# starreeze/drin

Measured on AMD Instinct MI355X. Metric: mention x candidate pairs scored/sec, higher is better.
Workload: dtype bf16x3; 1 GPU; wikimel-shaped scoring forward: 100-cand (+1 answer slot), D=768, R=2048, L=128, P=49, T=64 token-level entity text; parallelism=dp1 (mentions sharded, no collective)

## Files before the change

drin_amd/_lib.py:

```python
from __future__ import annotations

import ctypes as C
import os
from typing import Optional

_HERE = os.path.dirname(os.path.abspath(__file__))
LIB_PATH = os.environ.get("DRIN_LIB_PATH") or os.path.join(_HERE, "libdrin_hip.so")
MAX_LAYERS = 8
ABI_VERSION = 12

OK, E_SHAPE, E_NULL, E_ALIGN, E_WORKSPACE, E_HIP, E_UNSUPPORTED, E_INDEX = 0, -1, -2, -3, -4, -5, -6, -7
PREC_F32, PREC_BF16X3, PREC_BF16X3_ALL, PREC_BF16X3_IF16 = 0, 1, 3, 5
FEAT_F32, FEAT_BF16 = 0, 1
CACHE_F32, CACHE_MIXED_F16 = 0, 1
CACHE_FORMATS = {"f32": CACHE_F32, "mixed_f16": CACHE_MIXED_F16}
ACTIVATIONS = {"gelu": 1, "sigmoid": 2, "relu": 3, "tanh": 4, "silu": 5}

fp = C.POINTER(C.c_float)
ip = C.POINTER(C.c_int64)


class DrinConfigC(C.Structure):
    _fields_ = [
        ("batch", C.c_int32), ("num_candidates", C.c_int32), ("embed_dim", C.c_int32), ("image_dim", C.c_int32),
        ("mention_tokens", C.c_int32), ("image_regions", C.c_int32), ("mention_objects", C.c_int32),
        ("entity_objects", C.c_int32), ("entity_tokens", C.c_int32), ("mention_object_inner", C.c_int32),
        ("entity_image_inner", C.c_int32), ("entity_object_inner", C.c_int32), ("num_layers", C.c_int32),
        ("dynamic_edges", C.c_int32), ("edge_enabled", C.c_float * 4), ("layer_norm_eps", C.c_float),
        ("cosine_eps", C.c_float), ("miei_eps", C.c_float), ("clip_scale", C.c_float), ("precision", C.c_int32),
        ("num_entities", C.c_int32), ("vector_edges", C.c_int32), ("feature_dtype", C.c_int32),
        ("vertex_activation", C.c_int32), ("edge_activation", C.c_int32), ("cache_format", C.c_int32),
    ]


class DrinBatchC(C.Structure):
    _fields_ = [
        ("mention_text", C.c_void_p), ("mention_start", C.c_void_p), ("mention_end", C.c_void_p),
        ("mention_image", C.c_void_p), ("mention_object", C.c_void_p), ("mention_object_score", C.c_void_p),
        ("entity_text", C.c_void_p), ("entity_text_mask", C.c_void_p), ("entity_image", C.c_void_p),
        ("entity_object", C.c_void_p), ("entity_object_score", C.c_void_p), ("miet_similarity", C.c_void_p),
        ("mtei_similarity", C.c_void_p), ("entity_index", C.c_void_p), ("entity_text_cls", C.c_void_p),
        ("index_status", C.c_void_p),
    ]


class DrinLayerParamsC(C.Structure):
    _fields_ = [(n, C.c_void_p) for n in ("w_h", "b_h", "w_u", "b_u", "w_v", "b_v", "ln_weight", "ln_bias", "w_m", "b_m")]


class DrinParamsC(C.Structure):
    _fields_ = [(n, C.c_void_p) for n in (
        "w_mention_text", "b_mention_text", "w_entity_text", "b_entity_text",
        "w_mention_image", "b_mention_image", "w_entity_image", "b_entity_image")] + [("layer", DrinLayerParamsC * MAX_LAYERS)]


class DrinParamGradsC(C.Structure):
    _fields_ = DrinParamsC._fields_


class DrinInputGradsC(C.Structure):
    _fields_ = [(n, C.c_void_p) for n in (
        "mention_text", "mention_image", "mention_object", "mention_object_score", "entity_text", "entity_text_cls",
        "entity_image", "entity_object", "entity_object_score", "miet_similarity", "mtei_similarity", "scratch")] + [
        ("scratch_bytes", C.c_size_t)]


class DrinMelhiConfigC(C.Structure):
    _fields_ = [("batch", C.c_int32), ("num_candidates", C.c_int32), ("embed_dim", C.c_int32), ("image_dim", C.c_int32),
                ("mention_tokens", C.c_int32), ("image_regions", C.c_int32), ("precision", C.c_int32),
                ("cosine_eps", C.c_float), ("thres_tmim", C.c_float), ("thres_imie", C.c_float)]


class DrinMelhiBatchC(C.Structure):
    _fields_ = [(n, C.c_void_p) for n in (
        "mention_feature", "mention_mask", "start", "end", "mention_image", "entity_feature", "entity_image")]


MELHI_PARAMS = ("w_image_map_text", "b_image_map_text", "w_ih", "w_hh", "b_ih", "b_hh", "w_mention_final_map",
                "b_mention_final_map", "w_entity_final_map", "b_entity_final_map")


class DrinMelhiParamsC(C.Structure):
    _fields_ = [(n, C.c_void_p) for n in MELHI_PARAMS]


class DrinMelhiParamGradsC(C.Structure):
    _fields_ = DrinMelhiParamsC._fields_


class DrinGhmfcConfigC(C.Structure):
    _fields_ = [("batch", C.c_int32), ("num_candidates", C.c_int32), ("embed_dim", C.c_int32), ("image_dim", C.c_int32),
                ("mention_tokens", C.c_int32), ("image_regions", C.c_int32), ("num_heads", C.c_int32),
                ("entity_tokens", C.c_int32), ("precision", C.c_int32), ("layer_norm_eps", C.c_float), ("cosine_eps", C.c_float)]


class DrinGhmfcBatchC(C.Structure):
    _fields_ = [(n, C.c_void_p) for n in ("mention_feature", "mention_mask", "mention_image", "entity_feature", "entity_mask")]


GHMFC_CROSS_PARAMS = ("a2b_wq", "a2b_wk", "a2b_wv", "a2b_in_bias", "a2b_wo", "a2b_bo", "a2b_ffn_w", "a2b_ffn_b", "b2a_in_w",
                      "b2a_in_bias", "b2a_wo", "b2a_bo", "b2a_ffn_w", "b2a_ffn_b", "ln0_w", "ln0_b", "ln1_w", "ln1_b", "ln2_w",
                      "ln2_b", "ln3_w", "ln3_b")


class DrinGhmfcCrossParamsC(C.Structure):
    _fields_ = [(n, C.c_void_p) for n in GHMFC_CROSS_PARAMS]


class DrinGhmfcParamsC(C.Structure):
    _fields_ = [("t2v", DrinGhmfcCrossParamsC), ("v2t", DrinGhmfcCrossParamsC)] + [(n, C.c_void_p) for n in (
        "w_text_linear", "b_text_linear", "w_image_linear", "b_image_linear", "w_score_linear", "b_score_linear", "w_entity",
        "b_entity")]


class DrinTraceC(C.Structure):
    _fields_ = [(n, C.c_void_p * (MAX_LAYERS + 1)) for n in (
        "mention_text_vertex", "mention_image_vertex", "entity_text_vertex", "entity_image_vertex", "edges")]


EXPORTS = {
    "drin_version": (C.c_int, []),
    "drin_last_error": (C.c_char_p, []),
    "drin_build_info": (C.c_char_p, []),
    "drin_default_config": (C.c_int, [C.POINTER(DrinConfigC)]),
    "drin_host_selftest": (C.c_int, []),
    "drin_workspace_bytes": (C.c_size_t, [C.POINTER(DrinConfigC), C.c_int]),
    "drin_edges_fwd": (C.c_int, [C.POINTER(DrinConfigC), C.POINTER(DrinBatchC), C.c_void_p, C.c_void_p, C.c_void_p]),
    "drin_pool_fwd": (C.c_int, [C.POINTER(DrinConfigC), C.POINTER(DrinBatchC), C.c_void_p, C.c_void_p, C.c_void_p, C.c_void_p]),
    "drin_linear_fwd": (C.c_int, [C.c_void_p, C.c_void_p, C.c_void_p, C.c_void_p, C.c_int64, C.c_int32, C.c_int32, C.c_int32, C.c_void_p]),
    "drin_linear_bwd": (C.c_int, [C.c_void_p, C.c_void_p, C.c_void_p, C.c_void_p, C.c_void_p, C.c_void_p, C.c_int64, C.c_int32,
                                  C.c_int32, C.c_int32, C.c_void_p, C.c_size_t, C.c_void_p]),
    "drin_forward": (C.c_int, [C.POINTER(DrinConfigC), C.POINTER(DrinBatchC), C.POINTER(DrinParamsC), C.c_void_p,
                               C.c_size_t, C.c_void_p, C.c_int, C.POINTER(DrinTraceC), C.c_void_p]),
    "drin_forward_staged": (C.c_int, [C.POINTER(DrinConfigC), C.POINTER(DrinBatchC), C.POINTER(DrinParamsC), C.c_void_p,
                                      C.c_size_t, C.c_void_p, C.c_int, C.POINTER(DrinTraceC), C.c_void_p, C.c_void_p]),
    "drin_backward": (C.c_int, [C.POINTER(DrinConfigC), C.POINTER(DrinBatchC), C.POINTER(DrinParamsC), C.c_void_p,
                                C.c_size_t, C.c_void_p, C.POINTER(DrinParamGradsC), C.c_void_p]),
    "drin_backward_staged": (C.c_int, [C.POINTER(DrinConfigC), C.POINTER(DrinBatchC), C.POINTER(DrinParamsC), C.c_void_p,
                                       C.c_size_t, C.c_void_p, C.POINTER(DrinParamGradsC), C.c_void_p, C.c_void_p]),
    "drin_backward_ex": (C.c_int, [C.POINTER(DrinConfigC), C.POINTER(DrinBatchC), C.POINTER(DrinParamsC), C.c_void_p,
                                   C.c_size_t, C.c_void_p, C.POINTER(DrinParamGradsC), C.POINTER(DrinInputGradsC), C.c_void_p,
                                   C.c_void_p]),
    "drin_input_grad_scratch_bytes": (C.c_size_t, [C.POINTER(DrinConfigC)]),
    "drin_pool_bwd": (C.c_int, [C.POINTER(DrinConfigC), C.c_void_p, C.c_void_p, C.c_void_p, C.c_void_p, C.c_void_p]),
    "drin_fused_supported": (C.c_int, [C.POINTER(DrinConfigC)]),
    "drin_indexed_supported": (C.c_int, [C.POINTER(DrinConfigC)]),
    "drin_prepared_bytes": (C.c_size_t, [C.POINTER(DrinConfigC)]),
    "drin_fused_workspace_bytes": (C.c_size_t, [C.POINTER(DrinConfigC)]),
    "drin_workgroups_per_mention": (C.c_int32, [C.POINTER(DrinConfigC), C.c_int32]),
    "drin_index_status": (C.c_int, [C.c_void_p, C.c_void_p]),
    "drin_image_contraction_passes": (C.c_int32, [C.POINTER(DrinConfigC), C.c_int32]),
    "drin_prepare": (C.c_int, [C.POINTER(DrinConfigC), C.POINTER(DrinParamsC), C.c_void_p, C.c_size_t, C.c_void_p]),
    "drin_forward_prepared": (C.c_int, [C.POINTER(DrinConfigC), C.POINTER(DrinBatchC), C.POINTER(DrinParamsC), C.c_void_p,
                                        C.c_void_p, C.c_size_t, C.c_void_p, C.c_void_p]),
    "drin_entity_cache_bytes": (C.c_size_t, [C.POINTER(DrinConfigC)]),
    "drin_entity_cache_build_workspace_bytes": (C.c_size_t, [C.POINTER(DrinConfigC)]),
    "drin_cached_workspace_bytes": (C.c_size_t, [C.POINTER(DrinConfigC)]),
    "drin_build_entity_cache": (C.c_int, [C.POINTER(DrinConfigC), C.POINTER(DrinBatchC), C.POINTER(DrinParamsC), C.c_void_p,
                                          C.c_void_p, C.c_size_t, C.c_void_p, C.c_size_t, C.c_void_p]),
    "drin_forward_cached": (C.c_int, [C.POINTER(DrinConfigC), C.POINTER(DrinBatchC), C.POINTER(DrinParamsC), C.c_void_p,
                                      C.c_void_p, C.c_void_p, C.c_size_t, C.c_void_p, C.c_void_p]),
    "drin_split_planes": (C.c_int, [C.c_void_p, C.c_void_p, C.c_void_p, C.c_int64, C.c_void_p]),
    "drin_linear_planes_fwd": (C.c_int, [C.c_void_p, C.c_void_p, C.c_void_p, C.c_void_p, C.c_void_p, C.c_void_p,
                                         C.c_int64, C.c_int32, C.c_int32, C.c_void_p]),
    "drin_loss_workspace_bytes": (C.c_size_t, [C.c_int32]),
    "drin_triplet_topk": (C.c_int, [C.c_void_p, C.c_void_p, C.c_int32, C.c_int32, C.c_float, C.POINTER(C.c_int32), C.c_int32,
                                    C.c_void_p, C.c_void_p, C.c_void_p, C.c_void_p, C.c_size_t, C.c_void_p]),
    "drin_adam_step": (C.c_int, [C.c_void_p, C.c_void_p, C.c_void_p, C.c_void_p, C.c_int64, C.c_float, C.c_float, C.c_float,
                                 C.c_float, C.c_float, C.c_float, C.c_void_p]),
    "drin_melhi_workspace_bytes": (C.c_size_t, [C.POINTER(DrinMelhiConfigC), C.c_int]),
    "drin_melhi_forward": (C.c_int, [C.POINTER(DrinMelhiConfigC), C.POINTER(DrinMelhiBatchC), C.POINTER(DrinMelhiParamsC), C.c_void_p,
                                     C.c_void_p, C.c_void_p, C.c_size_t, C.c_void_p, C.c_void_p]),
    "drin_melhi_backward": (C.c_int, [C.POINTER(DrinMelhiConfigC), C.POINTER(DrinMelhiBatchC), C.POINTER(DrinMelhiParamsC),
                                      C.c_void_p, C.c_void_p, C.c_void_p, C.c_size_t, C.c_void_p, C.POINTER(DrinMelhiParamGradsC),
                                      C.c_void_p]),
    "drin_ghmfc_workspace_bytes": (C.c_size_t, [C.POINTER(DrinGhmfcConfigC)]),
    "drin_ghmfc_forward": (C.c_int, [C.POINTER(DrinGhmfcConfigC), C.POINTER(DrinGhmfcBatchC), C.POINTER(DrinGhmfcParamsC), C.c_void_p,
                                     C.c_size_t, C.c_void_p, C.c_void_p, C.c_void_p]),
    "drin_attention": (C.c_int, [C.c_void_p, C.c_int64, C.c_void_p, C.c_int64, C.c_void_p, C.c_int64, C.c_void_p, C.c_void_p, C.c_int64,
                                 C.c_int32, C.c_int32, C.c_int32, C.c_int32, C.c_int32, C.c_void_p]),
    "drin_attention_train_fwd": (C.c_int, [C.c_void_p, C.c_int64, C.c_void_p, C.c_int64, C.c_void_p, C.c_int64, C.c_void_p, C.c_void_p,
                                           C.c_int64, C.c_void_p, C.c_int32, C.c_int32, C.c_int32, C.c_int32, C.c_int32, C.c_void_p]),
    "drin_attention_bwd": (C.c_int, [C.c_void_p, C.c_int64, C.c_void_p, C.c_int64, C.c_void_p, C.c_int64, C.c_void_p, C.c_void_p,
                                     C.c_int64, C.c_void_p, C.c_void_p, C.c_int64, C.c_void_p, C.c_int64, C.c_void_p, C.c_int64,
                                     C.c_void_p, C.c_int64, C.c_void_p, C.c_int32, C.c_int32, C.c_int32, C.c_int32, C.c_int32,
                                     C.c_void_p]),
    "drin_profile_begin": (C.c_int, [C.c_int]),
    "drin_profile_end": (C.c_int, [C.POINTER(C.c_double), C.POINTER(C.c_int64)]),
    "drin_kernel_class_name": (C.c_char_p, [C.c_int]),
}
KERNEL_CLASSES = 12


class DrinError(RuntimeError):
    def __init__(self, status: int, message: str):
        super().__init__(f"libdrin_hip status {status}: {message}")
        self.status = status


_lib: Optional[C.CDLL] = None


def load() -> C.CDLL:
    global _lib
    if _lib is not None:
        return _lib
    if not os.path.exists(LIB_PATH):
        raise ImportError(
            f"{LIB_PATH} is missing: the DRIN HIP path has no fallback. Build it with `python -m drin_amd.build`."
        )
    try:
        import torch
    except ImportError:
        pass
    lib = C.CDLL(LIB_PATH)
    for name, (res, args) in EXPORTS.items():
        fn = getattr(lib, name)
        fn.restype, fn.argtypes = res, args
    if lib.drin_version() != ABI_VERSION:
        raise ImportError(f"libdrin_hip ABI {lib.drin_version()} != binding {ABI_VERSION}; rebuild")
    _lib = lib
    return lib


def profile_begin(max_launches: int = 65536) -> None:
    check(load().drin_profile_begin(max_launches))


def profile_end() -> dict:
    ms = (C.c_double * KERNEL_CLASSES)()
    n = (C.c_int64 * KERNEL_CLASSES)()
    check(load().drin_profile_end(ms, n))
    lib = load()
    return {lib.drin_kernel_class_name(k).decode(): (ms[k], n[k]) for k in range(KERNEL_CLASSES)}


def check(status: int) -> None:
    if status != OK:
        raise DrinError(status, load().drin_last_error().decode())
```

drin_amd/csrc/api.hip:

```cpp
#include <dlfcn.h>
#include <stdarg.h>
#include <stdlib.h>

#include <atomic>
#include <mutex>
#include <stdio.h>
#include <string.h>

#include "fused.h"
#include "internal.h"
#include "layout.h"

namespace drin {

static thread_local char g_err[512] = "";

void set_error(const char* fmt, ...) {
  va_list ap;
  va_start(ap, fmt);
  vsnprintf(g_err, sizeof(g_err), fmt, ap);
  va_end(ap);
}

int hip_fail(hipError_t e, const char* what) {
  set_error("%s: %s", what, hipGetErrorString(e));
  return DRIN_E_HIP;
}

static thread_local int g_call_device = -1;

int call_device() {
  if (g_call_device >= 0) return g_call_device;
  int dev = 0;
  if (hipGetDevice(&dev) != hipSuccess) dev = 0;
  return dev;
}

DeviceScope::DeviceScope(void* stream, const void* device_pointer, const char* entry_point)
    : status(DRIN_OK), prev(-1), dev(-1), outer(g_call_device), switched(false) {
  hipError_t e = hipGetDevice(&prev);
  if (e != hipSuccess) {
    (void)hipGetLastError();
    prev = -1;
    return;
  }
  dev = prev;
  if (stream != nullptr) {
    hipDevice_t d = 0;
    e = hipStreamGetDevice((hipStream_t)stream, &d);
    if (e != hipSuccess) {
      set_error("%s: hipStreamGetDevice: %s (is `stream` a hipStream_t?)", entry_point, hipGetErrorString(e));
      status = DRIN_E_HIP;
      return;
    }
    dev = (int)d;
  } else if (device_pointer != nullptr) {
    hipPointerAttribute_t attr;
    if (hipPointerGetAttributes(&attr, device_pointer) == hipSuccess && attr.type == hipMemoryTypeDevice)
      dev = attr.device;
    else
      (void)hipGetLastError();
  }
  if (dev != prev) {
    e = hipSetDevice(dev);
    if (e != hipSuccess) {
      set_error("%s: hipSetDevice(%d): %s", entry_point, dev, hipGetErrorString(e));
      status = DRIN_E_HIP;
      return;
    }
    switched = true;
  }
  g_call_device = dev;
}

DeviceScope::~DeviceScope() {
  if (status != DRIN_OK || prev < 0) return;
  g_call_device = outer;
  if (switched) (void)hipSetDevice(prev);
}

struct Roctx {
  int (*push)(const char*) = nullptr;
  int (*pop)() = nullptr;
  Roctx() {
    if (!getenv("DRIN_ROCTX")) return;
    void* h = dlopen("librocprofiler-sdk-roctx.so", RTLD_NOW | RTLD_GLOBAL);
    if (!h) h = dlopen("libroctx64.so", RTLD_NOW | RTLD_GLOBAL);
    if (!h) return;
    push = reinterpret_cast<int (*)(const char*)>(dlsym(h, "roctxRangePushA"));
    pop = reinterpret_cast<int (*)()>(dlsym(h, "roctxRangePop"));
    if (!push || !pop) push = nullptr, pop = nullptr;
  }
};
static const Roctx& roctx() {
  static const Roctx r;
  return r;
}
RoctxRange::RoctxRange(const char* name) : pushed(false) {
  const Roctx& r = roctx();
  if (r.push) {
    r.push(name);
    pushed = true;
  }
}
RoctxRange::~RoctxRange() {
  if (pushed) roctx().pop();
}

struct Profile {
  std::atomic<bool> open{false};
  int capacity = 0;
  std::atomic<int> used{0};
  hipEvent_t* start = nullptr;
  hipEvent_t* stop = nullptr;
  int* cls = nullptr;
};
static Profile g_prof;
static std::mutex g_prof_mutex;

KernelTimer::KernelTimer(int kernel_class, hipStream_t st) : slot(-1), stream(st) {
  Profile& p = g_prof;
  if (!p.open.load(std::memory_order_acquire)) return;
  const int s = p.used.fetch_add(1, std::memory_order_relaxed);
  if (s >= p.capacity) return;
  slot = s;
  p.cls[slot] = kernel_class;
  (void)hipEventRecord(p.start[slot], st);
}

KernelTimer::~KernelTimer() {
  if (slot >= 0) (void)hipEventRecord(g_prof.stop[slot], stream);
}

static void profile_free(Profile& p) {
  for (int i = 0; i < p.capacity; ++i) {
    if (p.start) (void)hipEventDestroy(p.start[i]);
    if (p.stop) (void)hipEventDestroy(p.stop[i]);
  }
  delete[] p.start;
  delete[] p.stop;
  delete[] p.cls;
  p.start = p.stop = nullptr;
  p.cls = nullptr;
  p.capacity = 0;
  p.used.store(0);
  p.open.store(false);
}

int vertex_act(const drin_config* c) { return c->vertex_activation == DRIN_ACT_DEFAULT ? DRIN_ACT_GELU : c->vertex_activation; }
int edge_act(const drin_config* c) { return c->edge_activation == DRIN_ACT_DEFAULT ? DRIN_ACT_SIGMOID : c->edge_activation; }

int validate_config(const drin_config* c) {
  if (!c) {
    set_error("config is NULL");
    return DRIN_E_NULL;
  }
  if (c->batch < 0 || c->num_candidates <= 0 || c->embed_dim <= 0 || c->image_dim <= 0 || c->mention_tokens <= 0 ||
      c->image_regions <= 0 || c->mention_objects < 0 || c->entity_objects < 0 || c->entity_tokens < 0 ||
      c->mention_object_inner < 0 || c->entity_image_inner < 0 || c->entity_object_inner < 0) {
    set_error("config: negative or zero dimension");
    return DRIN_E_SHAPE;
  }
  if (c->embed_dim % 4 || c->image_dim % 4) {
    set_error("config: embed_dim=%d and image_dim=%d must be multiples of 4 (16-byte lane accesses)", c->embed_dim,
              c->image_dim);
    return DRIN_E_SHAPE;
  }
  if (c->embed_dim > 1024) {
    set_error("config: embed_dim=%d > 1024 is not built (LayerNorm row kept in registers)", c->embed_dim);
    return DRIN_E_UNSUPPORTED;
  }
  if (c->vector_edges && (c->embed_dim % 8)) {
    set_error("config: vector edges need embed_dim %% 8 == 0 (got %d)", c->embed_dim);
    return DRIN_E_SHAPE;
  }
  if (c->num_layers < 0 || c->num_layers > DRIN_MAX_LAYERS) {
    set_error("config: num_layers=%d outside [0, %d]", c->num_layers, DRIN_MAX_LAYERS);
    return DRIN_E_SHAPE;
  }
  if ((int64_t)c->batch * c->num_candidates > (int64_t)1 << 30) {
    set_error("config: batch * num_candidates too large for one call; split the batch");
    return DRIN_E_SHAPE;
  }
  if (c->feature_dtype != DRIN_FEAT_F32 && c->feature_dtype != DRIN_FEAT_BF16) {
    set_error("config: feature_dtype %d is not DRIN_FEAT_F32 / DRIN_FEAT_BF16", c->feature_dtype);
    return DRIN_E_UNSUPPORTED;
  }
  if (c->vertex_activation < DRIN_ACT_DEFAULT || c->vertex_activation > DRIN_ACT_SILU) {
    set_error("config: vertex_activation %d is not a drin_activation", c->vertex_activation);
    return DRIN_E_UNSUPPORTED;
  }
  if (c->edge_activation < DRIN_ACT_DEFAULT || c->edge_activation > DRIN_ACT_SILU) {
    set_error("config: edge_activation %d is not a drin_activation", c->edge_activation);
    return DRIN_E_UNSUPPORTED;
  }
  if (c->cache_format != DRIN_CACHE_F32 && c->cache_format != DRIN_CACHE_MIXED_F16) {
    set_error("config: cache_format %d is not a drin_cache_format", c->cache_format);
    return DRIN_E_UNSUPPORTED;
  }
  if (c->precision != DRIN_PREC_F32 && c->precision != DRIN_PREC_BF16X3 && c->precision != DRIN_PREC_BF16X3_ALL &&
      c->precision != DRIN_PREC_BF16X3_IF16) {
    set_error("config: precision %d is not a drin_precision", c->precision);
    return DRIN_E_UNSUPPORTED;
  }
  return DRIN_OK;
}

static int validate_batch(const drin_config* c, const drin_batch* b) {
  if (!b) {
    set_error("batch is NULL");
    return DRIN_E_NULL;
  }
  if (c->feature_dtype != DRIN_FEAT_F32) {
    set_error("bf16 feature storage is read by drin_forward_prepared only; widen the features to fp32 for this entry point");
    return DRIN_E_UNSUPPORTED;
  }
  if (c->precision == DRIN_PREC_BF16X3_IF16) {
    set_error("DRIN_PREC_BF16X3_IF16 (the entity-image contraction in one fp16 pass) is an inference mode of drin_forward_prepared; use DRIN_PREC_BF16X3 here");
    return DRIN_E_UNSUPPORTED;
  }
  const void* req[] = {b->mention_text,  b->mention_start,        b->mention_end,     b->mention_image,
                       b->mention_object, b->mention_object_score, b->entity_text,     b->entity_image,
                       b->entity_object,  b->entity_object_score,  b->miet_similarity, b->mtei_similarity};
  const char* names[] = {"mention_text",   "mention_start",        "mention_end",     "mention_image",
                         "mention_object", "mention_object_score", "entity_text",     "entity_image",
                         "entity_object",  "entity_object_score",  "miet_similarity", "mtei_similarity"};
  for (int i = 0; i < 12; ++i) {
    if (!req[i]) {
      set_error("batch.%s is NULL", names[i]);
      return DRIN_E_NULL;
    }
  }
  if (c->entity_tokens > 0 && !b->entity_text_mask) {
    set_error("batch.entity_text_mask is NULL but entity_tokens=%d", c->entity_tokens);
    return DRIN_E_NULL;
  }
  if (b->entity_text_cls && c->entity_tokens > 0) {
    set_error("batch.entity_text_cls goes with pooled entity text (entity_tokens = 0), not with a token block");
    return DRIN_E_UNSUPPORTED;
  }
  const void* al[] = {b->mention_text, b->mention_image, b->mention_object, b->entity_text, b->entity_image,
                      b->entity_object, b->entity_text_cls};
  for (const void* p : al)
    if (!aligned16(p)) {
      set_error("batch: feature tensors must be 16-byte aligned");
      return DRIN_E_ALIGN;
    }
  return DRIN_OK;
}

static int validate_params(const drin_config* c, const drin_params* p) {
  if (!p) {
    set_error("params is NULL");
    return DRIN_E_NULL;
  }
  const void* req[] = {p->w_mention_text,  p->b_mention_text,  p->w_entity_text,  p->b_entity_text,
                       p->w_mention_image, p->b_mention_image, p->w_entity_image, p->b_entity_image};
  for (const void* q : req)
    if (!q || !aligned16(q)) {
      set_error("params: vertex encoder tensor NULL or not 16-byte aligned");
      return q ? DRIN_E_ALIGN : DRIN_E_NULL;
    }
  for (int l = 0; l < c->num_layers; ++l) {
    const drin_layer_params& L = p->layer[l];
    const void* lr[] = {L.w_h, L.b_h, L.w_u, L.b_u, L.w_v, L.b_v, L.ln_weight, L.ln_bias};
    for (const void* q : lr)
      if (!q || !aligned16(q)) {
        set_error("params: layer %d tensor NULL or not 16-byte aligned", l);
        return q ? DRIN_E_ALIGN : DRIN_E_NULL;
      }
    if (c->vector_edges && (!L.w_m || !L.b_m || !aligned16(L.w_m) || !aligned16(L.b_m))) {
      set_error("params: layer %d w_m / b_m (vector edges, model.py:112) NULL or not 16-byte aligned", l);
      return DRIN_E_NULL;
    }
  }
  return DRIN_OK;
}

static Pooled unpooled(const drin_config* c, const drin_batch* b, const float* span_mean) {
  Pooled p;
  p.span_mean = span_mean;
  p.mention_object = b->mention_object;
  p.entity_object = b->entity_object;
  p.entity_image = b->entity_image;
  p.entity_text = b->entity_text;
  p.entity_text_raw_stride = c->entity_tokens > 0 ? (int64_t)c->entity_tokens * c->embed_dim : c->embed_dim;
  return p;
}

void resolve_pooled(const drin_config* c, const drin_batch* b, const Layout& L, float* ws, Pooled* out) {
  *out = unpooled(c, b, ws + L.span_mean);
  out->mention_image = ws + L.mimg_pool;
  if (c->mention_object_inner > 1) out->mention_object = ws + L.mobj_pool;
  if (c->entity_object_inner > 1) out->entity_object = ws + L.eobj_pool;
  if (c->entity_image_inner > 1) out->entity_image = ws + L.eimg_pool;
  if (c->entity_tokens > 0) out->entity_text = ws + L.xet_pool;
}

int run_pooling(const drin_config* c, const drin_batch* b, const Layout& L, float* ws, Pooled* out, hipStream_t st) {
  const int B = c->batch, N = c->num_candidates, D = c->embed_dim, R = c->image_dim;
  const int64_t M = (int64_t)B * N;
  resolve_pooled(c, b, L, ws, out);
  auto copy_of = [](const float* resolved, const float* raw) { return resolved != raw ? const_cast<float*>(resolved) : nullptr; };
  DRIN_TRY(launch_span_mean(b->mention_text, b->mention_start, b->mention_end, ws + L.span_mean, B, c->mention_tokens, D, st));
  DRIN_TRY(launch_axis_mean(b->mention_image, ws + L.mimg_pool, B, c->image_regions, R, st));
  if (float* dst = copy_of(out->mention_object, b->mention_object))
    DRIN_TRY(launch_axis_mean(b->mention_object, dst, (int64_t)B * c->mention_objects, c->mention_object_inner, R, st));
  if (float* dst = copy_of(out->entity_object, b->entity_object))
    DRIN_TRY(launch_axis_mean(b->entity_object, dst, M * c->entity_objects, c->entity_object_inner, R, st));
  if (float* dst = copy_of(out->entity_image, b->entity_image))
    DRIN_TRY(launch_axis_mean(b->entity_image, dst, M, c->entity_image_inner, R, st));
  if (float* dst = copy_of(out->entity_text, b->entity_text))
    DRIN_TRY(launch_entity_token_mean(b->entity_text, b->entity_text_mask, dst, M, c->entity_tokens, D, st));
  return DRIN_OK;
}

int run_static_edges(const drin_config* c, const drin_batch* b, const Pooled& P, float* edges, hipStream_t st) {
  const int B = c->batch, N = c->num_candidates;
  const int64_t M = (int64_t)B * N;
  const float* raw = b->entity_text_cls ? b->entity_text_cls : b->entity_text;
  const int64_t raw_stride = b->entity_text_cls ? (int64_t)c->embed_dim : P.entity_text_raw_stride;
  DRIN_TRY(launch_cosine_rows(P.span_mean, raw, raw_stride, edges + 0 * M, B, N, c->embed_dim, c->cosine_eps, 1.0f, st,
                              b->entity_index, b->mtei_similarity, b->miet_similarity, edges + 1 * M, edges + 2 * M,
                              c->clip_scale));
  DRIN_TRY(launch_miei(P.mention_object, b->mention_object_score, P.entity_object, b->entity_object_score,
                       edges + 3 * M, B, N, c->mention_objects, c->entity_objects, c->image_dim, c->cosine_eps,
                       c->miei_eps, 1.0f, st, b->entity_index));
  return DRIN_OK;
}

static int copy_out(float* dst, const float* src, size_t n, hipStream_t st) {
  if (!dst) return DRIN_OK;
  hipError_t e = hipMemcpyAsync(dst, src, n * sizeof(float), hipMemcpyDeviceToDevice, st);
  if (e != hipSuccess) return hip_fail(e, "hipMemcpyAsync(trace)");
  return DRIN_OK;
}

static int tap(const drin_trace* t, int l, const Layout& L, const float* ws, int B, int64_t M, int D, hipStream_t st,
               size_t edge_width = 1) {
  if (!t) return DRIN_OK;
  DRIN_TRY(copy_out(t->mention_text_vertex[l], ws + L.vm[l], (size_t)B * D, st));
  DRIN_TRY(copy_out(t->mention_image_vertex[l], ws + L.vm[l] + (size_t)B * D, (size_t)B * D, st));
  DRIN_TRY(copy_out(t->entity_text_vertex[l], ws + L.ve[l], (size_t)M * D, st));
  DRIN_TRY(copy_out(t->entity_image_vertex[l], ws + L.ve[l] + (size_t)M * D, (size_t)M * D, st));
  DRIN_TRY(copy_out(t->edges[l], ws + L.edges[l], (size_t)4 * M * edge_width, st));
  return DRIN_OK;
}

static int indexed_supported(const drin_config* c, const char* who) {
  const int64_t M = (int64_t)c->batch * c->num_candidates;
  const int D = c->embed_dim, R = c->image_dim;
  const bool x3 = c->precision == DRIN_PREC_BF16X3 || c->precision == DRIN_PREC_BF16X3_ALL;
  if (c->num_entities <= 0 || c->entity_tokens != 0 || c->entity_image_inner > 1 || c->entity_object_inner > 1 ||
      c->entity_objects != 1 || c->vector_edges || !x3 || M < 1024 || (D % 32) || (R % 32) || D < 128 || R < 128 ||
      R > 2048 || c->batch > 65535) {
    set_error("%s: entity_index needs pooled entity text tables (entity_tokens = 0, num_entities > 0), one object per entity, "
              "inner dims <= 1, scalar edges, split-bf16 precision, D and R multiples of 32 (>= 128, R <= 2048) and at least "
              "1024 pairs; gather on the caller side otherwise", who);
    return DRIN_E_UNSUPPORTED;
  }
  return DRIN_OK;
}

struct InputGradScratch {
  size_t total_floats = 0;
  size_t g_span = 0, g_raw = 0, cls_stage = 0, g_pool = 0, cos3 = 0, g_mimg = 0, g_eimg = 0, g_mobj = 0, g_eobj = 0;
  size_t g_ms = 0, g_es = 0, g_edge = 0, planes_ei = 0, planes_et = 0, miei = 0;
  size_t take(size_t n) {
    const size_t o = total_floats;
    total_floats += (n + 63) & ~(size_t)63;
    return o;
  }
  void build(const drin_config& c) {
    const size_t B = (size_t)c.batch, N = (size_t)c.num_candidates, D = (size_t)c.embed_dim, R = (size_t)c.image_dim;
    const size_t M = B * N, Km = (size_t)c.mention_objects, Ke = (size_t)c.entity_objects;
    const bool x3 = c.precision == DRIN_PREC_BF16X3 || c.precision == DRIN_PREC_BF16X3_ALL;
    total_floats = 0;
    g_span = take(B * D);
    g_raw = take(M * D);
    cls_stage = take(c.entity_tokens > 0 ? M * D : 0);
    g_pool = take(c.entity_tokens > 0 ? M * D : 0);
// ... 870 lines not shown
```

drin_amd/csrc/fused_forward.hip:

```cpp
#include <string.h>

#include "fused.h"
#include "internal.h"
#include "layout.h"

namespace drin {

constexpr int kMixedMinCandidates = 64;

struct FusedLayout {
  size_t span_mean, mimg, vm0, hmfu, q, e0m, e1m, xt, s_part, s_text, s_img, sig, tm, tm2, agg1, vm1, hm2, h_text, h_image,
      et1, s2_part, agg2, mt2, p_xt, p_xi, p_et1, xi_scale, splitk, splitk_floats, pair_splitk, pair_splitk_floats, total;
  int chunks;
  void build(const drin_config& c) {
    const size_t B = c.batch, N = c.num_candidates, D = c.embed_dim, R = c.image_dim, M = B * N;
    chunks = (int)(B >= 2048 ? (N + 127) / 128 : B >= 1024 ? (N + 47) / 48 : (N + 15) / 16);
    size_t off = 0;
    auto take = [&off](size_t n) {
      const size_t o = off;
      off += (n + 63) & ~(size_t)63;
      return o;
    };
    span_mean = take(B * D);
    mimg = take(B * R);
    vm0 = take(2 * B * D);
    hmfu = take(2 * B * 2 * D);
    q = take(2 * B * (D + R));
    e0m = take(4 * M);
    e1m = take(4 * M);
    xt = take(c.entity_tokens > 0 ? M * D : 0);
    s_part = take(B * chunks * (2 * D + 2 * R + 4));
    s_text = take(2 * B * D);
    s_img = take(2 * B * R);
    sig = take(4 * B);
    tm = take(2 * B * D);
    tm2 = take(2 * B * D);
    agg1 = take(2 * B * D);
    vm1 = take(2 * B * D);
    hm2 = take(2 * B * D);
    h_text = take(M * D);
    h_image = take(M * D);
    et1 = take(M * D);
    s2_part = take(B * chunks * 2 * D);
    agg2 = take(B * D);
    mt2 = take(B * D);
    const bool planes = c.precision == DRIN_PREC_BF16X3 || c.precision == DRIN_PREC_BF16X3_ALL || c.precision == DRIN_PREC_BF16X3_IF16;
    p_xt = take(planes ? M * D : 0);
    p_xi = take(!planes ? 0 : c.num_entities > 0 ? M * R : c.precision == DRIN_PREC_BF16X3_IF16 ? M * R / 2 : 0);
    p_et1 = take(planes ? M * D : 0);
    xi_scale = take(c.precision == DRIN_PREC_BF16X3_IF16 ? M : 0);
    splitk_floats = 2 * B <= 512 ? 8 * 2 * B * (D + R) : 0;
    if (planes && splitk_floats < (size_t)192 * 65536) splitk_floats = (size_t)192 * 65536;
    splitk = take(splitk_floats);
    pair_splitk_floats = 0;
    {
      const size_t tiles = ((M + 255) / 256) * ((D + 255) / 256);
      if (planes && tiles <= 128)
        for (size_t s : {16, 8, 6, 4, 3, 2})
          if (tiles * s <= 256) {
            pair_splitk_floats = s * ((M + 255) / 256 * 256) * D;
            break;
          }
    }
    pair_splitk = take(pair_splitk_floats);
    total = off;
  }
};

static bool if16_gate(const drin_config* c, bool indexed) {
  const int64_t M = (int64_t)c->batch * c->num_candidates;
  return c->precision == DRIN_PREC_BF16X3_IF16 && !indexed && c->feature_dtype == DRIN_FEAT_F32 &&
         c->num_candidates >= kMixedMinCandidates && c->embed_dim == 768 && c->image_dim == 2048 &&
         cdiv(M, 256) * cdiv(c->embed_dim, 256) >= 128;
}

int fused_supported(const drin_config* c) {
  if (c->num_layers != 2) {
    set_error("fused path: built for num_layers == 2 (got %d); use drin_forward", c->num_layers);
    return DRIN_E_UNSUPPORTED;
  }
  if (c->vector_edges) {
    set_error("fused path: vector edge features (model.py:112-116) run on the layer-by-layer path; use drin_forward");
    return DRIN_E_UNSUPPORTED;
  }
  if (c->mention_object_inner > 1 || c->entity_object_inner > 1 || c->entity_image_inner > 1) {
    set_error("fused path: inner feature dims > 1 need the pooled path of drin_forward");
    return DRIN_E_UNSUPPORTED;
  }
  const bool tiny = c->embed_dim <= 256 && c->image_dim <= 256;
  const bool full = c->embed_dim <= 768 && c->image_dim <= 2048;
  if (!tiny && !full) {
    set_error("fused path: D=%d R=%d outside the built instantiations", c->embed_dim, c->image_dim);
    return DRIN_E_UNSUPPORTED;
  }
  return DRIN_OK;
}

}

using namespace drin;

extern "C" {

int drin_split_planes(const float* x, void* hi, void* lo, int64_t n, void* stream) {
  DRIN_BIND_DEVICE(stream, x, "drin_split_planes");
  if (!x || !hi || !lo) {
    set_error("drin_split_planes: NULL argument");
    return DRIN_E_NULL;
  }
  return launch_split_planes(x, hi, lo, n, (hipStream_t)stream);
}

int drin_linear_planes_fwd(const void* x_hi, const void* x_lo, const void* w_hi, const void* w_lo, const float* bias,
                           float* y, int64_t rows, int32_t n_out, int32_t k, void* stream) {
  DRIN_BIND_DEVICE(stream, y, "drin_linear_planes_fwd");
  if (!x_hi || !w_hi || !w_lo || !y) {
    set_error("drin_linear_planes_fwd: NULL argument");
    return DRIN_E_NULL;
  }
  return launch_gemm_x3_planes(x_hi, x_lo, k, w_hi, w_lo, k, bias, y, n_out, rows, n_out, k, (hipStream_t)stream);
}

int drin_fused_supported(const drin_config* cfg) {
  DRIN_TRY(validate_config(cfg));
  return fused_supported(cfg);
}

size_t drin_prepared_bytes(const drin_config* cfg) {
  if (validate_config(cfg) != DRIN_OK || fused_supported(cfg) != DRIN_OK) return 0;
  Prepared P;
  P.build(*cfg);
  return P.total * sizeof(float);
}

int drin_prepare(const drin_config* cfg, const drin_params* params, void* prepared, size_t prepared_bytes,
                 void* stream) {
  DRIN_BIND_DEVICE(stream, prepared, "drin_prepare");
  RoctxRange range("drin_prepare");
  DRIN_TRY(validate_config(cfg));
  DRIN_TRY(fused_supported(cfg));
  if (!params || !prepared) {
    set_error("drin_prepare: NULL argument");
    return DRIN_E_NULL;
  }
  Prepared P;
  P.build(*cfg);
  if (prepared_bytes < P.total * sizeof(float) || !aligned16(prepared)) {
    set_error("drin_prepare: buffer has %zu bytes (needs %zu) or is not 16-byte aligned", prepared_bytes,
              P.total * sizeof(float));
    return DRIN_E_WORKSPACE;
  }
  hipStream_t st = (hipStream_t)stream;
  float* pb = (float*)prepared;
  const int D = cfg->embed_dim, R = cfg->image_dim;
  const drin_layer_params& L1 = params->layer[0];
  const int F32 = DRIN_PREC_F32;
  auto copy = [&](float* dst, const float* src, size_t n) -> int {
    hipError_t e = hipMemcpyAsync(dst, src, n * sizeof(float), hipMemcpyDeviceToDevice, st);
    return e == hipSuccess ? DRIN_OK : hip_fail(e, "hipMemcpyAsync(prepare)");
  };
  DRIN_TRY(copy(pb + P.wcat1, L1.w_h, (size_t)D * D));
  DRIN_TRY(copy(pb + P.wcat1 + (size_t)D * D, L1.w_u, (size_t)D * D));
  {
    hipError_t e = hipMemsetAsync(pb + P.bcat1, 0, D * sizeof(float), st);
    if (e != hipSuccess) return hip_fail(e, "hipMemsetAsync(prepare)");
  }
  DRIN_TRY(copy(pb + P.bcat1 + D, L1.b_u, D));
  DRIN_TRY(launch_gemm_nn(L1.w_v, D, params->w_entity_text, D, pb + P.etmp, D + R, D, D, D, false, F32, st));
  DRIN_TRY(launch_gemm_nn(L1.w_v, D, params->w_entity_image, R, pb + P.etmp + D, D + R, D, R, D, false, F32, st));
  DRIN_TRY(launch_transpose(pb + P.etmp, pb + P.ecat, D, D + R, st));
  DRIN_TRY(launch_gemm_nt(params->b_entity_text, D, L1.w_v, D, L1.b_v, pb + P.k_t, D, 1, D, D, false, F32, st));
  DRIN_TRY(launch_gemm_nt(params->b_entity_image, D, L1.w_v, D, L1.b_v, pb + P.k_i, D, 1, D, D, false, F32, st));
  DRIN_TRY(launch_gemm_nn(L1.w_h, D, params->w_entity_text, D, pb + P.c_txt, D, D, D, D, false, F32, st));
  DRIN_TRY(launch_gemm_nn(L1.w_h, D, params->w_entity_image, R, pb + P.c_img, R, D, R, D, false, F32, st));
  DRIN_TRY(launch_gemm_nt(params->b_entity_text, D, L1.w_h, D, L1.b_h, pb + P.cb_t, D, 1, D, D, false, F32, st));
  DRIN_TRY(launch_gemm_nt(params->b_entity_image, D, L1.w_h, D, L1.b_h, pb + P.cb_i, D, 1, D, D, false, F32, st));
  {
    const size_t dd = (size_t)D * D, dr = (size_t)D * R;
    __bf16* q = reinterpret_cast<__bf16*>(pb + P.p_ctxt);
    DRIN_TRY(launch_split_planes(pb + P.c_txt, q, q + dd, dd, st));
    q = reinterpret_cast<__bf16*>(pb + P.p_cimg);
    DRIN_TRY(launch_split_planes(pb + P.c_img, q, q + dr, dr, st));
    DRIN_TRY(launch_to_f16_scaled(pb + P.c_img, pb + P.p_cimg_f16, (int64_t)dr, pb + P.cimg_f16_scale, st));
    q = reinterpret_cast<__bf16*>(pb + P.p_wh2);
    DRIN_TRY(launch_split_planes(params->layer[1].w_h, q, q + dd, dd, st));
    struct { size_t off; const float* w; size_t n; } extra[] = {
        {P.p_wmt, params->w_mention_text, dd},  {P.p_wmi, params->w_mention_image, dr},
        {P.p_wcat1, pb + P.wcat1, 2 * dd},      {P.p_ecat, pb + P.ecat, dd + dr},
        {P.p_wet, params->w_entity_text, dd},   {P.p_wei, params->w_entity_image, dr},
        {P.p_wh1, L1.w_h, dd}};
    for (const auto& e : extra) {
      q = reinterpret_cast<__bf16*>(pb + e.off);
      DRIN_TRY(launch_split_planes(e.w, q, q + e.n, e.n, st));
    }
  }
  return DRIN_OK;
}

}

namespace drin {

static int folded_precision(const drin_config* c) { return c->precision == DRIN_PREC_BF16X3_IF16 ? (int)DRIN_PREC_BF16X3 : c->precision; }

int run_folded_head(const drin_config* cfg, const drin_batch* b, const drin_params* params, const float* pb, const Prepared& P,
                    bool weight_planes, float* span_mean, float* mimg, float* vm0, float* hmfu, GemmScratch sk, hipStream_t st) {
  const int B = cfg->batch, D = cfg->embed_dim, R = cfg->image_dim, prec = folded_precision(cfg);
  auto wp = [&](size_t plane_off) -> const float* { return weight_planes ? pb + plane_off : nullptr; };
  if (cfg->feature_dtype == DRIN_FEAT_BF16) {
    DRIN_TRY(launch_span_mean_bf16(b->mention_text, b->mention_start, b->mention_end, span_mean, B, cfg->mention_tokens, D, st));
    DRIN_TRY(launch_axis_mean_bf16(b->mention_image, mimg, B, cfg->image_regions, R, st));
  } else {
    DRIN_TRY(launch_span_mean(b->mention_text, b->mention_start, b->mention_end, span_mean, B, cfg->mention_tokens, D, st));
    DRIN_TRY(launch_axis_mean(b->mention_image, mimg, B, cfg->image_regions, R, st));
  }
  DRIN_TRY(launch_gemm_nt_pair({span_mean, params->w_mention_text, params->b_mention_text, vm0, D, D, D, B, D, D, wp(P.p_wmt)},
                               {mimg, params->w_mention_image, params->b_mention_image, vm0 + (size_t)B * D, R, R, D, B, D, R, wp(P.p_wmi)},
                               prec, st, sk.p, sk.floats));
  return launch_gemm_nt(vm0, D, pb + P.wcat1, D, pb + P.bcat1, hmfu, 2 * D, 2 * (int64_t)B, 2 * D, D, false, prec, st, sk.p, sk.floats,
                        wp(P.p_wcat1));
}

int run_folded_mention_finish(const drin_config* cfg, const drin_params* params, const float* pb, const Prepared& P,
                              bool weight_planes, float* vm1, float* hm2, GemmScratch sk, hipStream_t st) {
  const int B = cfg->batch, D = cfg->embed_dim;
  const drin_layer_params& L1 = params->layer[0];
  DRIN_TRY(launch_layernorm_gelu(vm1, L1.ln_weight, L1.ln_bias, vm1, nullptr, nullptr, 2 * (int64_t)B, D, cfg->layer_norm_eps, st,
                                 vertex_act(cfg)));
  return launch_gemm_nt(vm1, D, params->layer[1].w_h, D, nullptr, hm2, D, 2 * (int64_t)B, D, D, false, folded_precision(cfg), st, sk.p,
                        sk.floats, weight_planes ? pb + P.p_wh2 : nullptr);
}

int run_folded_tail(const drin_config* cfg, const drin_params* params, const float* pb, const Prepared& P, int chunks,
                    const float* s2_part, const float* vm1, float* agg2, float* mt2, const float* hm2, const float* e1m, float* h2,
                    const float* et1, const void* et1_hi, bool weight_planes, GemmScratch sk, GemmScratch pair_sk, float* scores,
                    hipStream_t st) {
  const int B = cfg->batch, N = cfg->num_candidates, D = cfg->embed_dim, prec = folded_precision(cfg);
  const int64_t M = (int64_t)B * N;
  const drin_layer_params& L2 = params->layer[1];
  DRIN_TRY(launch_mention_input2(s2_part, vm1, agg2, B, D, N, chunks, st));
  DRIN_TRY(launch_gemm_nt(agg2, D, L2.w_h, D, L2.b_h, mt2, D, B, D, D, false, prec, st, sk.p, sk.floats,
                          weight_planes ? pb + P.p_wh2 : nullptr));
  DRIN_TRY(launch_layernorm_gelu(mt2, L2.ln_weight, L2.ln_bias, mt2, nullptr, nullptr, B, D, cfg->layer_norm_eps, st, vertex_act(cfg)));
  if (et1_hi) {
    const __bf16* e1 = static_cast<const __bf16*>(et1_hi);
    const __bf16* w2 = reinterpret_cast<const __bf16*>(pb + P.p_wh2);
    DRIN_TRY(launch_gemm_x3_planes(e1, e1 + (size_t)M * D, D, w2, w2 + (size_t)D * D, D, nullptr, h2, D, M, D, D, st, pair_sk.p,
                                   pair_sk.floats));
  } else {
    DRIN_TRY(launch_gemm_nt(et1, D, L2.w_h, D, nullptr, h2, D, M, D, D, false, prec, st));
  }
  FinalArgs fa = shaped_args<FinalArgs>(*cfg);
  set_vertex_fields(fa, *cfg);
  fa.h2 = h2;
  fa.hm2 = hm2;
  fa.b_h2 = L2.b_h;
  fa.gamma = L2.ln_weight;
  fa.beta = L2.ln_bias;
  fa.e1m = e1m;
  fa.mt2 = mt2;
  fa.scores = scores;
  fa.chunks = chunks;
  fa.cos_eps = cfg->cosine_eps;
  return launch_pair_final(fa, st);
}

static int forward_prepared_on_stream(const drin_config* cfg, const drin_batch* b, const drin_params* params, const void* prepared,
                                      void* workspace, float* scores, hipStream_t st) {
  FusedLayout L;
  L.build(*cfg);
  Prepared P;
  P.build(*cfg);
  float* ws = (float*)workspace;
  const float* pb = (const float*)prepared;
  const int B = cfg->batch, N = cfg->num_candidates, D = cfg->embed_dim, R = cfg->image_dim;
  const int64_t M = (int64_t)B * N;
  if (B == 0) return DRIN_OK;
  const int prec = folded_precision(cfg);
  const bool dyn = cfg->dynamic_edges != 0;
  const bool tokens = cfg->entity_tokens > 0;
  const bool planes = (prec == DRIN_PREC_BF16X3 || prec == DRIN_PREC_BF16X3_ALL) && (D % 32 == 0) && (R % 32 == 0);
  const bool indexed = b->entity_index != nullptr;
  const bool xi_planes = planes && indexed;
  const bool if16 = if16_gate(cfg, indexed) && gemm_f16_planes_fits(ws + L.p_xi, R, pb + P.p_cimg_f16, R, ws + L.h_image, D, M, D, R);
  if (b->entity_text_cls) {
    set_error("drin_forward_prepared: entity_text_cls (text pooled ahead of time) is a form of the training entry points");
    return DRIN_E_UNSUPPORTED;
  }
  if (indexed && cfg->num_entities <= 0) {
    set_error("drin_forward_prepared: entity_index given but cfg.num_entities = %d", cfg->num_entities);
    return DRIN_E_SHAPE;
  }
  if (indexed && !planes) {
    set_error("drin_forward_prepared: entity_index needs the split-bf16 precision (the stream kernel gathers the "
              "GEMM operands as planes); gather on the caller side for DRIN_PREC_F32");
    return DRIN_E_UNSUPPORTED;
  }
  const bool bf16_feat = cfg->feature_dtype == DRIN_FEAT_BF16;
  if (bf16_feat && !planes) {
    set_error("drin_forward_prepared: bf16 features need the split-bf16 precision (DRIN_PREC_BF16X3) and D, R multiples of 32");
    return DRIN_E_UNSUPPORTED;
  }
  __bf16* xt_hi = reinterpret_cast<__bf16*>(ws + L.p_xt);
  __bf16* xi_hi = reinterpret_cast<__bf16*>(ws + L.p_xi);
  __bf16* e1_hi = reinterpret_cast<__bf16*>(ws + L.p_et1);
  const size_t MD = (size_t)M * D, MR = (size_t)M * R;
  const drin_layer_params& L1 = params->layer[0];

  auto wp = [&](size_t plane_off) -> const float* { return planes ? pb + plane_off : nullptr; };
  const GemmScratch msk{L.splitk_floats ? ws + L.splitk : nullptr, L.splitk_floats};
  float* vm0 = ws + L.vm0;
  float* hmfu = ws + L.hmfu;
  const bool xt_exact = bf16_feat && !tokens;
  DRIN_TRY(run_folded_head(cfg, b, params, pb, P, planes, ws + L.span_mean, ws + L.mimg, vm0, hmfu, msk, st));
  if (dyn)
    DRIN_TRY(launch_gemm_nt(hmfu + D, 2 * D, pb + P.ecat, D, nullptr, ws + L.q, D + R, 2 * (int64_t)B, D + R, D, false, prec, st, msk.p,
                            msk.floats, wp(P.p_ecat)));
  StreamArgs sa = shaped_args<StreamArgs>(*cfg);
  set_edge_fields(sa, *cfg);
  sa.entity_text = b->entity_text;
  sa.entity_mask = b->entity_text_mask;
  sa.entity_image = b->entity_image;
  sa.entity_object = b->entity_object;
  sa.entity_object_score = b->entity_object_score;
  sa.entity_index = b->entity_index;
  sa.num_entities = cfg->num_entities;
  sa.index_status = b->index_status;
  sa.miet = b->miet_similarity;
  sa.mtei = b->mtei_similarity;
  sa.span_mean = ws + L.span_mean;
  sa.mobj = b->mention_object;
  sa.mscore = b->mention_object_score;
  sa.fu = hmfu + D;
  sa.ldfu = 2 * D;
  sa.q = ws + L.q;
  sa.ldq = D + R;
  sa.k_t = pb + P.k_t;
  sa.k_i = pb + P.k_i;
  sa.xt_out = planes ? nullptr : ws + L.xt;
  if (planes) {
    sa.xt_hi = xt_hi;
    sa.xt_lo = xt_exact ? nullptr : xt_hi + MD;
    if (xi_planes) {
      sa.xi_hi = xi_hi;
      sa.xi_lo = bf16_feat ? nullptr : xi_hi + MR;
    }
  }
  sa.xi_scale = if16 ? ws + L.xi_scale : nullptr;
  sa.xi_f16 = if16 ? static_cast<void*>(xi_hi) : nullptr;
  sa.e0m = ws + L.e0m;
  sa.e1m = ws + L.e1m;
  sa.s_part = ws + L.s_part;
  sa.T = cfg->entity_tokens;
  sa.Ke = cfg->entity_objects;
  sa.chunks = L.chunks;
  sa.bf16_features = bf16_feat ? 1 : 0;
  sa.s_text = ws + L.s_text;
  sa.s_img = ws + L.s_img;
  sa.sig = ws + L.sig;
  DRIN_TRY(launch_entity_stream(sa, st));
  if (L.chunks > 1)
    DRIN_TRY(launch_reduce_stream_partials(ws + L.s_part, ws + L.s_text, ws + L.s_img, ws + L.sig, B, D, R, L.chunks, st));
  DRIN_TRY(launch_gemm_nt_pair({ws + L.s_text, params->w_entity_text, nullptr, ws + L.tm, D, D, D, 2 * (int64_t)B, D, D, wp(P.p_wet)},
                               {ws + L.s_img, params->w_entity_image, nullptr, ws + L.tm2, R, R, D, 2 * (int64_t)B, D, R,
                                wp(P.p_wei)},
                               prec, st, msk.p, msk.floats));
  DRIN_TRY(launch_mention_input1(ws + L.tm, ws + L.tm2, ws + L.sig, params->b_entity_text, params->b_entity_image, vm0, ws + L.agg1, B, D, N, st));
  float* vm1 = ws + L.vm1;
  DRIN_TRY(launch_gemm_nt(ws + L.agg1, D, L1.w_h, D, L1.b_h, vm1, D, 2 * (int64_t)B, D, D, false, prec, st, msk.p, msk.floats, wp(P.p_wh1)));
  DRIN_TRY(run_folded_mention_finish(cfg, params, pb, P, planes, vm1, ws + L.hm2, msk, st));
  const GemmScratch psk = L.pair_splitk_floats ? GemmScratch{ws + L.pair_splitk, L.pair_splitk_floats} : msk;
  if (planes) {
    const __bf16* ct = reinterpret_cast<const __bf16*>(pb + P.p_ctxt);
    const __bf16* ci = reinterpret_cast<const __bf16*>(pb + P.p_cimg);
    DRIN_TRY(launch_gemm_x3_planes(xt_hi, xt_exact ? nullptr : xt_hi + MD, D, ct, ct + (size_t)D * D, D, nullptr, ws + L.h_text, D, M, D,
                                   D, st, psk.p, psk.floats));
    if (if16)
      DRIN_TRY(launch_gemm_f16_planes(xi_hi, R, pb + P.p_cimg_f16, R, ws + L.xi_scale, pb + P.cimg_f16_scale, ws + L.h_image, D, M, D, R,
                                      st, psk.p, psk.floats));
    else if (xi_planes)
      DRIN_TRY(launch_gemm_x3_planes(xi_hi, bf16_feat ? nullptr : xi_hi + MR, R, ci, ci + (size_t)D * R, R, nullptr, ws + L.h_image, D, M,
                                     D, R, st, psk.p, psk.floats));
    else if (bf16_feat)
      DRIN_TRY(launch_gemm_x3_planes(b->entity_image, nullptr, R, ci, ci + (size_t)D * R, R, nullptr, ws + L.h_image, D, M, D, R, st, psk.p,
                                     psk.floats));
    else
      DRIN_TRY(launch_gemm_nt_bf16x3(b->entity_image, R, pb + P.c_img, R, nullptr, ws + L.h_image, D, M, D, R, st, ci, ci + (size_t)D * R,
                                     false, psk.p, psk.floats));
  } else {
    const float* x_t = tokens ? ws + L.xt : b->entity_text;
    DRIN_TRY(launch_gemm_nt(x_t, D, pb + P.c_txt, D, nullptr, ws + L.h_text, D, M, D, D, false, prec, st));
    DRIN_TRY(launch_gemm_nt(b->entity_image, R, pb + P.c_img, R, nullptr, ws + L.h_image, D, M, D, R, false, prec, st));
  }
  PairArgs pa = shaped_args<PairArgs>(*cfg);
  set_vertex_fields(pa, *cfg);
  pa.h_text = ws + L.h_text;
  pa.h_image = ws + L.h_image;
  pa.hm = hmfu;
  pa.ldhm = 2 * D;
  pa.c_t = pb + P.cb_t;
  pa.c_i = pb + P.cb_i;
  pa.gamma = L1.ln_weight;
  pa.beta = L1.ln_bias;
  pa.e0m = ws + L.e0m;
  pa.e1m = ws + L.e1m;
  pa.et1 = planes ? nullptr : ws + L.et1;
  if (planes) {
    pa.et1_hi = e1_hi;
    pa.et1_lo = e1_hi + MD;
  }
  pa.s2_part = ws + L.s2_part;
  pa.chunks = L.chunks;
  DRIN_TRY(launch_pair_layer1(pa, st));
  return run_folded_tail(cfg, params, pb, P, L.chunks, ws + L.s2_part, vm1, ws + L.agg2, ws + L.mt2, ws + L.hm2, ws + L.e1m, ws + L.h_text,
                         planes ? nullptr : ws + L.et1, planes ? e1_hi : nullptr, planes, msk, psk, scores, st);
}

}

extern "C" {

int32_t drin_workgroups_per_mention(const drin_config* cfg, int32_t cached) {
  if (validate_config(cfg) != DRIN_OK || fused_supported(cfg) != DRIN_OK) return 0;
  if (cached) return cached_chunks_per_mention(*cfg);
  FusedLayout L;
  L.build(*cfg);
  return L.chunks;
}

int32_t drin_image_contraction_passes(const drin_config* cfg, int32_t indexed) {
  if (validate_config(cfg) != DRIN_OK || fused_supported(cfg) != DRIN_OK) return 0;
  if (cfg->precision == DRIN_PREC_F32) return 0;
  if (if16_gate(cfg, indexed != 0)) return 1;
  return cfg->feature_dtype == DRIN_FEAT_BF16 ? 2 : 3;
}

int drin_index_status(int32_t* index_status, void* stream) {
  if (!index_status) {
    set_error("drin_index_status: NULL argument");
    return DRIN_E_NULL;
  }
  DRIN_BIND_DEVICE(stream, index_status, "drin_index_status");
  int32_t w[4] = {0, 0, 0, 0};
  hipError_t e = hipMemcpyAsync(w, index_status, sizeof(w), hipMemcpyDeviceToHost, (hipStream_t)stream);
  if (e == hipSuccess) e = hipStreamSynchronize((hipStream_t)stream);
  if (e != hipSuccess) return hip_fail(e, "drin_index_status");
  if (w[0] == 0) return DRIN_OK;
  e = hipMemsetAsync(index_status, 0, sizeof(w), (hipStream_t)stream);
  if (e != hipSuccess) return hip_fail(e, "drin_index_status(reset)");
  const long long value = (long long)(((uint64_t)(uint32_t)w[3] << 32) | (uint32_t)w[2]);
  set_error("entity_index out of range: candidate row %lld at pair %d (b * N + n) is outside the entity tables - the row was clamped "
            "and a WRONG entity scored; drin/data.py:87-93 raises IndexError here", value, (int)w[1]);
  return DRIN_E_INDEX;
}

size_t drin_fused_workspace_bytes(const drin_config* cfg) {
  if (validate_config(cfg) != DRIN_OK || fused_supported(cfg) != DRIN_OK) return 0;
  FusedLayout L;
  L.build(*cfg);
  return L.total * sizeof(float);
}

int drin_forward_prepared(const drin_config* cfg, const drin_batch* b, const drin_params* params, const void* prepared,
                          void* workspace, size_t workspace_bytes, float* scores, void* stream) {
  DRIN_BIND_DEVICE(stream, workspace, "drin_forward_prepared");
  RoctxRange range("drin_forward_prepared");
  DRIN_TRY(validate_config(cfg));
  DRIN_TRY(fused_supported(cfg));
  if (!b || !params || !prepared || !workspace || !scores) {
    set_error("drin_forward_prepared: NULL argument");
    return DRIN_E_NULL;
  }
  FusedLayout L;
  L.build(*cfg);
  if (workspace_bytes < L.total * sizeof(float) || !aligned16(workspace)) {
    set_error("drin_forward_prepared: workspace has %zu bytes (needs %zu) or is not 16-byte aligned", workspace_bytes,
              L.total * sizeof(float));
    return DRIN_E_WORKSPACE;
  }
  return forward_prepared_on_stream(cfg, b, params, prepared, workspace, scores, (hipStream_t)stream);
}

}
```

drin_amd/csrc/gemm_x3_planes.hip:

```cpp
#include <stdlib.h>

#include "device_utils.h"
#include "internal.h"

namespace drin {

typedef float f32x16 __attribute__((ext_vector_type(16)));
typedef __bf16 bf16x8 __attribute__((ext_vector_type(8)));

namespace x3p {

constexpr int BM = 256, BN = 256, BK = 32;
constexpr int THREADS = 512;
constexpr int PLANE_BYTES = 256 * 64;
constexpr int BUF_BYTES = 4 * PLANE_BYTES;
constexpr int LDS_BYTES = 2 * BUF_BYTES;

__device__ __forceinline__ void tile_of_block(int& tile_x, int64_t& tile_y, int nx, unsigned full, int ksplit, int& kpart,
                                              unsigned& tail_slot) {
  const unsigned id = blockIdx.x;
  unsigned t;
  kpart = 0;
  tail_slot = 0;
  if (id < full) {
    const unsigned xcd = id & 7, k = id >> 3;
    const unsigned q = full >> 3, rem = full & 7;
    t = (xcd < rem ? xcd * (q + 1) : rem * (q + 1) + (xcd - rem) * q) + k;
  } else {
    const unsigned u = id - full;
    t = full + u / (unsigned)ksplit;
    kpart = (int)(u % (unsigned)ksplit);
    tail_slot = (u / (unsigned)ksplit) * (unsigned)(ksplit - 1) + (unsigned)(kpart - 1);
  }
  tile_x = (int)(t % (unsigned)nx);
  tile_y = (int64_t)(t / (unsigned)nx);
}

typedef __attribute__((address_space(1))) const void* gptr_t;
typedef __attribute__((address_space(3))) void* lptr_t;

struct Pieces {
  const char* base;
  int64_t ld_bytes;
  int64_t row0, lim;
};

template <bool A_LO, bool B_LO>
__device__ __forceinline__ void issue_piece(const Pieces& p, char* buf, int kb, int i) {
  const int wave = threadIdx.x >> 6;
  if (!A_LO && (wave >> 1) == 1) return;
  if (!B_LO && (wave >> 1) == 3) return;
  char* plane_base = buf + (wave >> 1) * PLANE_BYTES + (wave & 1) * 128 * 64;
  int64_t g = p.row0 + 16 * i;
  g = g < p.lim ? g : p.lim - 1;
  __builtin_amdgcn_global_load_lds((gptr_t)(p.base + g * p.ld_bytes + (int64_t)kb * (BK * 2)), (lptr_t)(plane_base + i * 1024),
                                   16, 0, 0);
}
template <bool A_LO, bool B_LO>
__device__ __forceinline__ void issue_tile(const Pieces& p, char* buf, int kb) {
#pragma unroll
  for (int i = 0; i < 8; ++i) issue_piece<A_LO, B_LO>(p, buf, kb, i);
}

typedef float f32x4 __attribute__((ext_vector_type(4)));

__device__ __forceinline__ int swz16(int row, int c) {
  const int f = (0x78 >> (((row >> 2) & 3) << 1)) & 3;
  return row * 64 + ((c ^ f) << 4);
}

__device__ __forceinline__ Pieces make_pieces(const __bf16* a_hi, const __bf16* a_lo, int64_t lda, int64_t m0,
                                                int64_t M, const __bf16* b_hi, const __bf16* b_lo, int64_t ldb,
                                                int64_t n0, int64_t N) {
  const int wave = threadIdx.x >> 6, lane = threadIdx.x & 63;
  const int plane = wave >> 1;
  const __bf16* base = plane == 0 ? a_hi : plane == 1 ? a_lo : plane == 2 ? b_hi : b_lo;
  const int64_t ld = plane < 2 ? lda : ldb, r0 = plane < 2 ? m0 : n0, lim = plane < 2 ? M : N;
  const int f = (0x78 >> (((lane >> 4) & 3) << 1)) & 3;
  const int chunk = (lane & 3) ^ f;
  Pieces p;
  p.base = reinterpret_cast<const char*>(base) + chunk * 16;
  p.ld_bytes = ld * 2;
  p.row0 = r0 + (wave & 1) * 128 + (lane >> 2);
  p.lim = lim;
  return p;
}

template <bool A_LO, bool B_LO>
__global__ void __launch_bounds__(THREADS, 2)
    k_gemm_x3_planes(const __bf16* __restrict__ a_hi, const __bf16* __restrict__ a_lo, int64_t lda,
                       const __bf16* __restrict__ b_hi, const __bf16* __restrict__ b_lo, int64_t ldb,
                       const float* __restrict__ bias, float* __restrict__ C, int64_t ldc, int64_t M, int N, int K,
                       int64_t part_stride, int nx, unsigned full, int ksplit, float* __restrict__ tail) {
  extern __shared__ __attribute__((aligned(16))) char smem[];
  if (gridDim.z > 1) {
    K /= (int)gridDim.z;
    const int64_t k0 = (int64_t)blockIdx.z * K;
    a_hi += k0;
    if (A_LO) a_lo += k0;
    b_hi += k0;
    if (B_LO) b_lo += k0;
    C += (int64_t)blockIdx.z * part_stride;
    ldc = N;
    bias = nullptr;
  }
  int tx, kpart;
  int64_t ty;
  unsigned tail_slot;
  tile_of_block(tx, ty, nx, full, ksplit, kpart, tail_slot);
  const int64_t m0 = ty * BM;
  const int n0 = tx * BN;
  if (blockIdx.x >= full) {
    K /= ksplit;
    const int64_t k0 = (int64_t)kpart * K;
    a_hi += k0;
    if (A_LO) a_lo += k0;
    b_hi += k0;
    if (B_LO) b_lo += k0;
  }
  const int nkb = K / BK;
  const int wave = threadIdx.x >> 6, lane = threadIdx.x & 63;
  const int wm = wave >> 2, wn = wave & 3;
  const int r = lane & 15, c = lane >> 4;

  f32x4 acc[8][4];
#pragma unroll
  for (int i = 0; i < 8; ++i)
#pragma unroll
    for (int j = 0; j < 4; ++j)
#pragma unroll
      for (int v = 0; v < 4; ++v) acc[i][j][v] = 0.f;

  const Pieces pieces = make_pieces(a_hi, A_LO ? a_lo : a_hi, lda, m0, M, b_hi, B_LO ? b_lo : b_hi, ldb, n0, N);
  issue_tile<A_LO, B_LO>(pieces, smem, 0);
  __syncthreads();

  for (int kb = 0; kb < nkb; ++kb) {
    const int cur = kb & 1;
    const char* buf = smem + cur * BUF_BYTES;
    const bool more = kb + 1 < nkb;
    char* nbuf = smem + (cur ^ 1) * BUF_BYTES;
    bf16x8 bh[4], bl[4], ah[2], al[2];
#pragma unroll
    for (int j = 0; j < 4; ++j) {
      const int off = swz16(wn * 64 + j * 16 + r, c);
      bh[j] = *reinterpret_cast<const bf16x8*>(buf + 2 * PLANE_BYTES + off);
      if (B_LO) bl[j] = *reinterpret_cast<const bf16x8*>(buf + 3 * PLANE_BYTES + off);
    }
    {
      const int off = swz16(wm * 128 + r, c);
      ah[0] = *reinterpret_cast<const bf16x8*>(buf + off);
      if (A_LO) al[0] = *reinterpret_cast<const bf16x8*>(buf + PLANE_BYTES + off);
    }
#pragma unroll
    for (int t = 0; t < 8; ++t) {
      if (more) issue_piece<A_LO, B_LO>(pieces, nbuf, kb + 1, t);
      if (t + 1 < 8) {
        const int off = swz16(wm * 128 + (t + 1) * 16 + r, c);
        ah[(t + 1) & 1] = *reinterpret_cast<const bf16x8*>(buf + off);
        if (A_LO) al[(t + 1) & 1] = *reinterpret_cast<const bf16x8*>(buf + PLANE_BYTES + off);
      }
      if (A_LO) {
#pragma unroll
        for (int j = 0; j < 4; ++j) acc[t][j] = __builtin_amdgcn_mfma_f32_16x16x32_bf16(bh[j], al[t & 1], acc[t][j], 0, 0, 0);
      }
      if (B_LO) {
#pragma unroll
        for (int j = 0; j < 4; ++j) acc[t][j] = __builtin_amdgcn_mfma_f32_16x16x32_bf16(bl[j], ah[t & 1], acc[t][j], 0, 0, 0);
      }
#pragma unroll
      for (int j = 0; j < 4; ++j) acc[t][j] = __builtin_amdgcn_mfma_f32_16x16x32_bf16(bh[j], ah[t & 1], acc[t][j], 0, 0, 0);
    }
    __syncthreads();
  }

  if (kpart > 0) {
    float* part = tail + (size_t)tail_slot * (BM * BN);
#pragma unroll
    for (int i = 0; i < 8; ++i)
#pragma unroll
      for (int j = 0; j < 4; ++j)
        st4(part + (wm * 128 + i * 16 + r) * BN + wn * 64 + j * 16 + c * 4,
            make_float4(acc[i][j][0], acc[i][j][1], acc[i][j][2], acc[i][j][3]));
    return;
  }
  const bool vec_ok = (ldc % 4) == 0 && (reinterpret_cast<uintptr_t>(C) & 15u) == 0;
#pragma unroll
  for (int i = 0; i < 8; ++i) {
    const int64_t row = m0 + wm * 128 + i * 16 + r;
    if (row >= M) continue;
#pragma unroll
    for (int j = 0; j < 4; ++j) {
      const int col = n0 + wn * 64 + j * 16 + c * 4;
      float* dst = C + row * ldc + col;
      if (vec_ok && col + 3 < N) {
        float4 o = make_float4(acc[i][j][0], acc[i][j][1], acc[i][j][2], acc[i][j][3]);
        if (bias != nullptr) o = o + ld4(bias + col);
        st4(dst, o);
      } else {
#pragma unroll
        for (int v = 0; v < 4; ++v)
          if (col + v < N) dst[v] = acc[i][j][v] + (bias != nullptr ? bias[col + v] : 0.f);
      }
    }
  }
}


__device__ __forceinline__ int pow2_exponent(float s) { return (int)((__builtin_bit_cast(uint32_t, s) >> 23) & 0xffu) - 127; }
__device__ __forceinline__ float4 scale_pow2(float4 v, int e) { return make_float4(ldexpf(v.x, e), ldexpf(v.y, e), ldexpf(v.z, e), ldexpf(v.w, e)); }

namespace p4 {

__device__ __forceinline__ void wait_units() { asm volatile("s_waitcnt vmcnt(4)" ::: "memory"); }
constexpr int UNIT_BYTES = 2 * 128 * 64;
constexpr int BUF = 4 * UNIT_BYTES;
constexpr int LDS = 2 * BUF;

struct Src {
  const char* ptr[4][2];
};

template <int U, int KB_BYTES = BK * 2>
__device__ __forceinline__ void issue_unit(const Src& s, char* buf, int kb) {
  const int wave = threadIdx.x >> 6;
  char* dst = buf + U * UNIT_BYTES + (wave >> 2) * (128 * 64) + (wave & 3) * 2048;
#pragma unroll
  for (int i = 0; i < 2; ++i)
    __builtin_amdgcn_global_load_lds((gptr_t)(s.ptr[U][i] + (int64_t)kb * KB_BYTES), (lptr_t)(dst + i * 1024), 16, 0, 0);
}

}

template <bool A_LO = true, bool F16 = false>
__global__ void __launch_bounds__(THREADS, 2)
    k_gemm_x3_planes_p4(const __bf16* __restrict__ a_hi, const __bf16* __restrict__ a_lo, int64_t lda,
                        const __bf16* __restrict__ b_hi, const __bf16* __restrict__ b_lo, int64_t ldb,
                        const float* __restrict__ bias, float* __restrict__ C, int64_t ldc, int64_t M, int N, int K, int nx,
                        unsigned full, int ksplit, float* __restrict__ tail, const float* __restrict__ row_scale,
                        const float* __restrict__ b_scale) {
  static_assert(!F16 || A_LO, "the fp16 form uses both slots of every unit");
  constexpr int KSTEP = F16 ? 2 * BK : BK;
  constexpr int KB_BYTES = KSTEP * 2;
  if (F16) {
    a_lo = a_hi + BK;
    b_lo = b_hi + BK;
  }
  extern __shared__ __attribute__((aligned(16))) char smem[];
  int tx, kpart;
  int64_t ty;
  unsigned tail_slot;
  tile_of_block(tx, ty, nx, full, ksplit, kpart, tail_slot);
  const int64_t m0 = ty * BM;
  const int n0 = tx * BN;
  int64_t k0 = 0;
  if (blockIdx.x >= full) {
    K /= ksplit;
    k0 = (int64_t)kpart * K;
  }
  const int nkb = K / KSTEP;
  const int wave = threadIdx.x >> 6, lane = threadIdx.x & 63;
  const int wm = wave >> 2, wn = wave & 3;
  const int r = lane & 15, c = lane >> 4;

  p4::Src src;
  {
    const int f = (0x78 >> (((lane >> 4) & 3) << 1)) & 3;
    const int chunk = (lane & 3) ^ f;
    const bool lo = wave >= 4;
    const char* ap = reinterpret_cast<const char*>((lo ? a_lo : a_hi) + k0) + chunk * 16;
    const char* bp = reinterpret_cast<const char*>((lo ? b_lo : b_hi) + k0) + chunk * 16;
#pragma unroll
    for (int u = 0; u < 4; ++u)
#pragma unroll
      for (int i = 0; i < 2; ++i) {
        const bool is_b = u >= 2;
        int64_t g = (is_b ? (int64_t)n0 : m0) + (u & 1) * 128 + (wave & 3) * 32 + 16 * i + (lane >> 2);
        const int64_t lim = is_b ? (int64_t)N : M;
        g = g < lim ? g : lim - 1;
        src.ptr[u][i] = (is_b ? bp : ap) + g * (is_b ? ldb : lda) * 2;
      }
  }

  f32x4 acc[2][2][4][2];
#pragma unroll
  for (int a = 0; a < 2; ++a)
#pragma unroll
    for (int b = 0; b < 2; ++b)
#pragma unroll
      for (int i = 0; i < 4; ++i)
#pragma unroll
        for (int j = 0; j < 2; ++j)
#pragma unroll
          for (int v = 0; v < 4; ++v) acc[a][b][i][j][v] = 0.f;

  bf16x8 ah[4], al[4], bh[2], bl[2];
  auto read_a = [&](const char* buf, int half) {
#pragma unroll
    for (int i = 0; i < 4; ++i) {
      const char* p = buf + half * p4::UNIT_BYTES + swz16(wm * 64 + i * 16 + r, c);
      ah[i] = *reinterpret_cast<const bf16x8*>(p);
      if (A_LO) al[i] = *reinterpret_cast<const bf16x8*>(p + 128 * 64);
    }
  };
  auto read_b = [&](const char* buf, int half) {
#pragma unroll
    for (int j = 0; j < 2; ++j) {
      const char* p = buf + (2 + half) * p4::UNIT_BYTES + swz16(wn * 32 + j * 16 + r, c);
      bh[j] = *reinterpret_cast<const bf16x8*>(p);
      bl[j] = *reinterpret_cast<const bf16x8*>(p + 128 * 64);
    }
  };
  auto mma = [&](f32x4 (&cc)[4][2]) {
    __builtin_amdgcn_s_setprio(1);
    if constexpr (F16) {
      typedef _Float16 f16x8 __attribute__((ext_vector_type(8)));
#pragma unroll
      for (int i = 0; i < 4; ++i)
#pragma unroll
        for (int j = 0; j < 2; ++j)
          cc[i][j] = __builtin_amdgcn_mfma_f32_16x16x32_f16(__builtin_bit_cast(f16x8, bh[j]), __builtin_bit_cast(f16x8, ah[i]), cc[i][j], 0, 0, 0);
#pragma unroll
      for (int i = 0; i < 4; ++i)
#pragma unroll
        for (int j = 0; j < 2; ++j)
          cc[i][j] = __builtin_amdgcn_mfma_f32_16x16x32_f16(__builtin_bit_cast(f16x8, bl[j]), __builtin_bit_cast(f16x8, al[i]), cc[i][j], 0, 0, 0);
      __builtin_amdgcn_s_setprio(0);
      return;
    }
    if (A_LO) {
#pragma unroll
      for (int i = 0; i < 4; ++i)
#pragma unroll
        for (int j = 0; j < 2; ++j) cc[i][j] = __builtin_amdgcn_mfma_f32_16x16x32_bf16(bh[j], al[i], cc[i][j], 0, 0, 0);
    }
#pragma unroll
    for (int i = 0; i < 4; ++i)
#pragma unroll
      for (int j = 0; j < 2; ++j) cc[i][j] = __builtin_amdgcn_mfma_f32_16x16x32_bf16(bl[j], ah[i], cc[i][j], 0, 0, 0);
#pragma unroll
    for (int i = 0; i < 4; ++i)
#pragma unroll
      for (int j = 0; j < 2; ++j) cc[i][j] = __builtin_amdgcn_mfma_f32_16x16x32_bf16(bh[j], ah[i], cc[i][j], 0, 0, 0);
    __builtin_amdgcn_s_setprio(0);
  };
  auto barrier = [&]() {
    __builtin_amdgcn_sched_barrier(0);
    __builtin_amdgcn_s_barrier();
    __builtin_amdgcn_sched_barrier(0);
  };
  p4::issue_unit<0, KB_BYTES>(src, smem, 0);
  p4::issue_unit<2, KB_BYTES>(src, smem, 0);
  p4::issue_unit<3, KB_BYTES>(src, smem, 0);
  p4::issue_unit<1, KB_BYTES>(src, smem, 0);
  asm volatile("s_waitcnt vmcnt(0)" ::: "memory");
  barrier();
  if (wm == 1) barrier();

#define P4_PHASE(READS, UNIT, ACC)                 \
  {                                                \
    READS;                                         \
    p4::issue_unit<UNIT, KB_BYTES>(src, nbuf, kn); \
    p4::wait_units();                              \
    barrier();                                     \
    mma(ACC);                                      \
    barrier();                                     \
  }
  for (int kb = 0; kb < nkb; ++kb) {
    const char* buf = smem + (kb & 1) * p4::BUF;
    char* nbuf = smem + ((kb + 1) & 1) * p4::BUF;
    const int kn = kb + 1 < nkb ? kb + 1 : kb;
    P4_PHASE((read_a(buf, 0), read_b(buf, 0)), 0, acc[0][0])
    P4_PHASE(read_b(buf, 1), 2, acc[0][1])
    P4_PHASE(read_a(buf, 1), 3, acc[1][1])
    P4_PHASE(read_b(buf, 0), 1, acc[1][0])
  }
#undef P4_PHASE
  asm volatile("s_waitcnt vmcnt(0)" ::: "memory");
  if (wm == 0) barrier();

  if (kpart > 0) {
    float* part = tail + (size_t)tail_slot * (BM * BN);
#pragma unroll
    for (int a = 0; a < 2; ++a)
#pragma unroll
      for (int i = 0; i < 4; ++i) {
        const int64_t row = m0 + a * 128 + wm * 64 + i * 16 + r;
        const int rs = F16 ? pow2_exponent(row_scale[row < M ? row : M - 1]) + pow2_exponent(*b_scale) : 0;
#pragma unroll
        for (int b = 0; b < 2; ++b)
#pragma unroll
          for (int j = 0; j < 2; ++j) {
            float4 o = make_float4(acc[a][b][i][j][0], acc[a][b][i][j][1], acc[a][b][i][j][2], acc[a][b][i][j][3]);
            if (F16) o = scale_pow2(o, rs);
            st4(part + (a * 128 + wm * 64 + i * 16 + r) * BN + b * 128 + wn * 32 + j * 16 + c * 4, o);
          }
      }
    return;
  }
  const int bs = F16 ? pow2_exponent(*b_scale) : 0;
  float4 bv[2][2];
#pragma unroll
  for (int b = 0; b < 2; ++b)
#pragma unroll
    for (int j = 0; j < 2; ++j) {
      const int col = n0 + b * 128 + wn * 32 + j * 16 + c * 4;
      bv[b][j] = (bias != nullptr && col < N) ? ld4(bias + col) : make_float4(0.f, 0.f, 0.f, 0.f);
    }
#pragma unroll
  for (int a = 0; a < 2; ++a)
#pragma unroll
    for (int i = 0; i < 4; ++i) {
      const int64_t row = m0 + a * 128 + wm * 64 + i * 16 + r;
      if (row >= M) continue;
      const int rs = F16 ? pow2_exponent(row_scale[row]) + bs : 0;
#pragma unroll
      for (int b = 0; b < 2; ++b)
#pragma unroll
        for (int j = 0; j < 2; ++j) {
          const int col = n0 + b * 128 + wn * 32 + j * 16 + c * 4;
          if (col >= N) continue;
          float4 o = make_float4(acc[a][b][i][j][0], acc[a][b][i][j][1], acc[a][b][i][j][2], acc[a][b][i][j][3]);
          if (F16) o = scale_pow2(o, rs);
          st4(C + row * ldc + col, o + bv[b][j]);
        }
    }
}


typedef float f32x4v __attribute__((ext_vector_type(4)));
typedef __bf16 bf16x4p __attribute__((ext_vector_type(4)));

__device__ __forceinline__ void split_store(f32x4v v, char* hi_plane, int off) {
  bf16x4p h, l;
  split_bf16x4(make_float4(v[0], v[1], v[2], v[3]), h, l);
  *reinterpret_cast<bf16x4p*>(hi_plane + off) = h;
  *reinterpret_cast<bf16x4p*>(hi_plane + 128 * 64 + off) = l;
}

__global__ void __launch_bounds__(THREADS, 2)
    k_gemm_bf16x3_p4(const float* __restrict__ A, int64_t lda, const __bf16* __restrict__ b_hi, const __bf16* __restrict__ b_lo,
                     int64_t ldb, const float* __restrict__ bias, float* __restrict__ C, int64_t ldc, int64_t M, int N, int K,
                     int accumulate, int nx, unsigned full, int ksplit, float* __restrict__ tail) {
  extern __shared__ __attribute__((aligned(16))) char smem[];
  int tx, kpart;
  int64_t ty;
  unsigned tail_slot;
  tile_of_block(tx, ty, nx, full, ksplit, kpart, tail_slot);
  const int64_t m0 = ty * BM;
  const int n0 = tx * BN;
  if (blockIdx.x >= full) {
    K /= ksplit;
    const int64_t k0 = (int64_t)kpart * K;
    A += k0;
    b_hi += k0;
    b_lo += k0;
  }
  const int nkb = K / BK;
  const int wave = threadIdx.x >> 6, lane = threadIdx.x & 63;
  const int wm = wave >> 2, wn = wave & 3;
  const int r = lane & 15, c = lane >> 4;

  p4::Src src;
  const float* arow[2][2];
  int a_off[2];
  {
    const int f = (0x78 >> (((lane >> 4) & 3) << 1)) & 3;
    const int chunk = (lane & 3) ^ f;
    const char* bp = reinterpret_cast<const char*>(wave >= 4 ? b_lo : b_hi) + chunk * 16;
#pragma unroll
    for (int u = 2; u < 4; ++u)
#pragma unroll
      for (int i = 0; i < 2; ++i) {
        int64_t g = (int64_t)n0 + (u & 1) * 128 + (wave & 3) * 32 + 16 * i + (lane >> 2);
        g = g < N ? g : (int64_t)N - 1;
        src.ptr[u][i] = bp + g * ldb * 2;
      }
    src.ptr[0][0] = src.ptr[0][1] = src.ptr[1][0] = src.ptr[1][1] = nullptr;
    const int c4 = threadIdx.x & 7;
    int urow[2];
#pragma unroll
    for (int i = 0; i < 2; ++i) urow[i] = (int)(threadIdx.x >> 8) * 64 + (int)((threadIdx.x & 255) >> 3) + 32 * i;
#pragma unroll
    for (int h = 0; h < 2; ++h)
#pragma unroll
      for (int i = 0; i < 2; ++i) {
        int64_t g = m0 + h * 128 + urow[i];
        g = g < M ? g : M - 1;
        arow[h][i] = A + g * lda + c4 * 4;
      }
#pragma unroll
    for (int i = 0; i < 2; ++i) a_off[i] = swz16(urow[i], c4 >> 1) + ((c4 & 1) << 3);
  }

  f32x4 acc[2][2][4][2];
#pragma unroll
  for (int a = 0; a < 2; ++a)
#pragma unroll
    for (int b = 0; b < 2; ++b)
#pragma unroll
      for (int i = 0; i < 4; ++i)
#pragma unroll
        for (int j = 0; j < 2; ++j)
#pragma unroll
          for (int v = 0; v < 4; ++v) acc[a][b][i][j][v] = 0.f;

  bf16x8 ah[4], al[4], bh[2], bl[2];
  auto read_a = [&](const char* buf, int half) {
#pragma unroll
    for (int i = 0; i < 4; ++i) {
      const char* p = buf + half * p4::UNIT_BYTES + swz16(wm * 64 + i * 16 + r, c);
      ah[i] = *reinterpret_cast<const bf16x8*>(p);
      al[i] = *reinterpret_cast<const bf16x8*>(p + 128 * 64);
    }
  };
  auto read_b = [&](const char* buf, int half) {
#pragma unroll
    for (int j = 0; j < 2; ++j) {
      const char* p = buf + (2 + half) * p4::UNIT_BYTES + swz16(wn * 32 + j * 16 + r, c);
      bh[j] = *reinterpret_cast<const bf16x8*>(p);
      bl[j] = *reinterpret_cast<const bf16x8*>(p + 128 * 64);
    }
  };
  auto mma_b = [&](f32x4 (&cc)[4][2], const bf16x8 (&fh)[2], const bf16x8 (&fl)[2]) {
    __builtin_amdgcn_s_setprio(1);
#pragma unroll
    for (int i = 0; i < 4; ++i)
#pragma unroll
      for (int j = 0; j < 2; ++j) cc[i][j] = __builtin_amdgcn_mfma_f32_16x16x32_bf16(fh[j], al[i], cc[i][j], 0, 0, 0);
#pragma unroll
    for (int i = 0; i < 4; ++i)
#pragma unroll
      for (int j = 0; j < 2; ++j) cc[i][j] = __builtin_amdgcn_mfma_f32_16x16x32_bf16(fl[j], ah[i], cc[i][j], 0, 0, 0);
#pragma unroll
    for (int i = 0; i < 4; ++i)
#pragma unroll
      for (int j = 0; j < 2; ++j) cc[i][j] = __builtin_amdgcn_mfma_f32_16x16x32_bf16(fh[j], ah[i], cc[i][j], 0, 0, 0);
    __builtin_amdgcn_s_setprio(0);
  };
  auto mma_split = [&](f32x4 (&cc)[4][2], const bf16x8 (&fh)[2], const bf16x8 (&fl)[2], char* dst_buf, int half, f32x4v v0, f32x4v v1) {
    __builtin_amdgcn_s_setprio(1);
#pragma unroll
    for (int i = 0; i < 4; ++i)
#pragma unroll
      for (int j = 0; j < 2; ++j) cc[i][j] = __builtin_amdgcn_mfma_f32_16x16x32_bf16(fh[j], al[i], cc[i][j], 0, 0, 0);
    split_store(v0, dst_buf + half * p4::UNIT_BYTES, a_off[0]);
#pragma unroll
    for (int i = 0; i < 4; ++i)
#pragma unroll
      for (int j = 0; j < 2; ++j) cc[i][j] = __builtin_amdgcn_mfma_f32_16x16x32_bf16(fl[j], ah[i], cc[i][j], 0, 0, 0);
    split_store(v1, dst_buf + half * p4::UNIT_BYTES, a_off[1]);
#pragma unroll
    for (int i = 0; i < 4; ++i)
#pragma unroll
      for (int j = 0; j < 2; ++j) cc[i][j] = __builtin_amdgcn_mfma_f32_16x16x32_bf16(fh[j], ah[i], cc[i][j], 0, 0, 0);
    __builtin_amdgcn_s_setprio(0);
    asm volatile("s_waitcnt lgkmcnt(0)" ::: "memory");
  };
  auto barrier = [&]() {
    __builtin_amdgcn_sched_barrier(0);
    __builtin_amdgcn_s_barrier();
    __builtin_amdgcn_sched_barrier(0);
  };
  auto load_a = [&](int half, int kb, f32x4v& v0, f32x4v& v1) {
    const float* p0 = arow[half][0] + (int64_t)kb * BK;
    const float* p1 = arow[half][1] + (int64_t)kb * BK;
    asm volatile("global_load_dwordx4 %0, %1, off" : "=v"(v0) : "v"(p0) : "memory");
    asm volatile("global_load_dwordx4 %0, %1, off" : "=v"(v1) : "v"(p1) : "memory");
  };
  auto wait4 = [&]() { p4::wait_units(); };
  auto landed = [&](f32x4v& v0, f32x4v& v1) { asm volatile("" : "+v"(v0), "+v"(v1) : : "memory"); };
  auto store_a = [&](char* buf, int half, f32x4v v0, f32x4v v1) {
    split_store(v0, buf + half * p4::UNIT_BYTES, a_off[0]);
    split_store(v1, buf + half * p4::UNIT_BYTES, a_off[1]);
    asm volatile("s_waitcnt lgkmcnt(0)" ::: "memory");
  };

  f32x4v a0v0, a0v1, a1v0, a1v1;
  load_a(0, 0, a0v0, a0v1);
  p4::issue_unit<2>(src, smem, 0);
  p4::issue_unit<3>(src, smem, 0);
  load_a(1, 0, a1v0, a1v1);
  asm volatile("s_waitcnt vmcnt(0)" ::: "memory");
  landed(a0v0, a0v1);
  landed(a1v0, a1v1);
  store_a(smem, 0, a0v0, a0v1);
  barrier();
  if (wm == 1) barrier();

  bf16x8 b0h[2], b0l[2];
  for (int kb = 0; kb < nkb; ++kb) {
    char* buf = smem + (kb & 1) * p4::BUF;
    char* nbuf = smem + ((kb + 1) & 1) * p4::BUF;
    const int kn = kb + 1 < nkb ? kb + 1 : kb;
    read_a(buf, 0);
#pragma unroll
    for (int j = 0; j < 2; ++j) {
      const char* p = buf + 2 * p4::UNIT_BYTES + swz16(wn * 32 + j * 16 + r, c);
      b0h[j] = *reinterpret_cast<const bf16x8*>(p);
      b0l[j] = *reinterpret_cast<const bf16x8*>(p + 128 * 64);
    }
    p4::issue_unit<2>(src, nbuf, kn);
    wait4();
    barrier();
    mma_b(acc[0][0], b0h, b0l);
    barrier();
    read_b(buf, 1);
    load_a(0, kn, a0v0, a0v1);
    wait4();
    landed(a1v0, a1v1);
    barrier();
    mma_split(acc[0][1], bh, bl, buf, 1, a1v0, a1v1);
    barrier();
    read_a(buf, 1);
    p4::issue_unit<3>(src, nbuf, kn);
    wait4();
    barrier();
    mma_b(acc[1][1], bh, bl);
    barrier();
    load_a(1, kn, a1v0, a1v1);
    wait4();
    landed(a0v0, a0v1);
    barrier();
    mma_split(acc[1][0], b0h, b0l, nbuf, 0, a0v0, a0v1);
    barrier();
  }
  asm volatile("s_waitcnt vmcnt(0)" ::: "memory");
  if (wm == 0) barrier();

  if (kpart > 0) {
    float* part = tail + (size_t)tail_slot * (BM * BN);
#pragma unroll
    for (int a = 0; a < 2; ++a)
#pragma unroll
      for (int i = 0; i < 4; ++i)
#pragma unroll
        for (int b = 0; b < 2; ++b)
#pragma unroll
          for (int j = 0; j < 2; ++j)
            st4(part + (a * 128 + wm * 64 + i * 16 + r) * BN + b * 128 + wn * 32 + j * 16 + c * 4,
                make_float4(acc[a][b][i][j][0], acc[a][b][i][j][1], acc[a][b][i][j][2], acc[a][b][i][j][3]));
    return;
  }
  float4 bv[2][2];
#pragma unroll
  for (int b = 0; b < 2; ++b)
#pragma unroll
    for (int j = 0; j < 2; ++j) {
      const int col = n0 + b * 128 + wn * 32 + j * 16 + c * 4;
      bv[b][j] = (bias != nullptr && col < N) ? ld4(bias + col) : make_float4(0.f, 0.f, 0.f, 0.f);
    }
#pragma unroll
  for (int a = 0; a < 2; ++a)
#pragma unroll
    for (int i = 0; i < 4; ++i) {
      const int64_t row = m0 + a * 128 + wm * 64 + i * 16 + r;
      if (row >= M) continue;
#pragma unroll
      for (int b = 0; b < 2; ++b)
#pragma unroll
        for (int j = 0; j < 2; ++j) {
          const int col = n0 + b * 128 + wn * 32 + j * 16 + c * 4;
          if (col >= N) continue;
          float* dst = C + row * ldc + col;
          float4 o = make_float4(acc[a][b][i][j][0], acc[a][b][i][j][1], acc[a][b][i][j][2], acc[a][b][i][j][3]) + bv[b][j];
          if (accumulate) o = o + ld4(dst);
          st4(dst, o);
        }
    }
}

__global__ void __launch_bounds__(256) k_split_planes(const float* __restrict__ x, __bf16* __restrict__ hi,
                                                      __bf16* __restrict__ lo, int64_t n4) {
  const int64_t i = (int64_t)blockIdx.x * 256 + threadIdx.x;
  if (i >= n4) return;
  const float4 v = ld4(x + i * 4);
  typedef __bf16 bf16x4 __attribute__((ext_vector_type(4)));
  bf16x4 h, l;
  split_bf16x4(v, h, l);
  *reinterpret_cast<bf16x4*>(hi + i * 4) = h;
  *reinterpret_cast<bf16x4*>(lo + i * 4) = l;
}

__global__ void __launch_bounds__(256) k_split_planes_batch(const SplitBatch b) {
  const int w = blockIdx.y;
  const int64_t n4 = b.n4[w];
  const float* __restrict__ x = b.src[w];
  __bf16* __restrict__ hi = reinterpret_cast<__bf16*>(b.planes[w]);
  __bf16* __restrict__ lo = hi + n4 * 4;
  typedef __bf16 bf16x4 __attribute__((ext_vector_type(4)));
  for (int64_t i = (int64_t)blockIdx.x * 256 + threadIdx.x; i < n4; i += (int64_t)gridDim.x * 256) {
    const float4 v = ld4(x + i * 4);
    bf16x4 h, l;
    split_bf16x4(v, h, l);
    *reinterpret_cast<bf16x4*>(hi + i * 4) = h;
    *reinterpret_cast<bf16x4*>(lo + i * 4) = l;
  }
}

__global__ void __launch_bounds__(256) k_transpose_split_batch(const SplitBatch b, int rows, int cols) {
  __shared__ float tile[32][33];
  const float* __restrict__ in = b.src[blockIdx.z];
  __bf16* __restrict__ hi = reinterpret_cast<__bf16*>(b.planes[blockIdx.z]);
  __bf16* __restrict__ lo = hi + (int64_t)rows * cols;
  const int tx = threadIdx.x & 31, ty = threadIdx.x >> 5;
  const int r0 = blockIdx.y * 32, c0 = blockIdx.x * 32;
  for (int i = ty; i < 32; i += 8)
    if (r0 + i < rows && c0 + tx < cols) tile[i][tx] = in[(int64_t)(r0 + i) * cols + c0 + tx];
  __syncthreads();
  for (int i = ty; i < 32; i += 8)
    if (c0 + i < cols && r0 + tx < rows) {
      const float v = tile[tx][i];
      const __bf16 h = (__bf16)v;
      const int64_t o = (int64_t)(c0 + i) * rows + r0 + tx;
      hi[o] = h;
      lo[o] = (__bf16)(v - (float)h);
    }
}

}


int launch_split_planes(const float* x, void* hi, void* lo, int64_t n, hipStream_t st) {
  if (n <= 0) return DRIN_OK;
  if (n % 4) {
    set_error("split_planes: element count %lld must be a multiple of 4", (long long)n);
    return DRIN_E_SHAPE;
  }
  KernelTimer timer(DRIN_KC_GCN, st);
  hipLaunchKernelGGL(x3p::k_split_planes, dim3((unsigned)cdiv(n / 4, 256)), dim3(256), 0, st, x, (__bf16*)hi,
                     (__bf16*)lo, n / 4);
  DRIN_CHECK_LAUNCH("k_split_planes");
  return DRIN_OK;
}

int SplitBatch::add(const float* w, float* planes_out, int64_t numel) {
  if (!w || numel <= 0) return DRIN_OK;
  if (n >= 32 || (numel % 4) || !aligned16(w) || !aligned16(planes_out)) {
    set_error("split_planes: at most 32 tensors per batch, element counts multiples of 4, 16-byte aligned");
    return DRIN_E_SHAPE;
  }
  src[n] = w, planes[n] = planes_out, n4[n] = numel / 4;
  ++n;
  return DRIN_OK;
}

int launch_split_planes_batch(const SplitBatch& b, hipStream_t st) {
  if (b.n == 0) return DRIN_OK;
  int64_t most = 0;
  for (int i = 0; i < b.n; ++i) most = most > b.n4[i] ? most : b.n4[i];
  int64_t gx = cdiv(most, 256);
  if (gx > 2048) gx = 2048;
  KernelTimer timer(DRIN_KC_GCN, st);
  hipLaunchKernelGGL(x3p::k_split_planes_batch, dim3((unsigned)gx, (unsigned)b.n), dim3(256), 0, st, b);
  DRIN_CHECK_LAUNCH("k_split_planes_batch");
  return DRIN_OK;
}

int launch_transpose_split_batch(const SplitBatch& b, int rows, int cols, hipStream_t st) {
  if (b.n == 0 || rows <= 0 || cols <= 0) return DRIN_OK;
  KernelTimer timer(DRIN_KC_GCN, st);
  hipLaunchKernelGGL(x3p::k_transpose_split_batch, dim3((unsigned)cdiv(cols, 32), (unsigned)cdiv(rows, 32), (unsigned)b.n), dim3(256),
                     0, st, b, rows, cols);
  DRIN_CHECK_LAUNCH("k_transpose_split_batch");
  return DRIN_OK;
}

static void tail_split_256(int64_t tiles, int nkb, const float* tail, size_t tail_floats, unsigned* full, int* ksplit) {
  *full = (unsigned)tiles;
  *ksplit = 1;
  if (tail == nullptr || !aligned16(tail) || tiles > 16 * 256) return;
  const unsigned frac = (unsigned)(tiles % 256);
  for (int s = 4; s >= 2 && frac > 0; --s)
    if ((unsigned)s * frac <= 256 && nkb % s == 0 && nkb / s >= 4 && (size_t)frac * (s - 1) * (x3p::BM * x3p::BN) <= tail_floats) {
      *ksplit = s;
      *full = (unsigned)tiles - frac;
      return;
    }
}

int launch_gemm_nt_bf16x3_p4(const float* x, int64_t ldx, const void* w_hi, const void* w_lo, int64_t ldw, const float* bias,
                             float* y, int64_t ldy, int64_t M, int N, int K, hipStream_t st, bool accumulate, float* tail,
                             size_t tail_floats) {
  if (M <= 0 || N <= 0) return DRIN_OK;
  if (K <= 0 || (K % x3p::BK) || (ldx % 4) || (ldw % 8) || (N % 4) || (ldy % 4) || !aligned16(x) || !aligned16(w_hi) || !aligned16(w_lo) ||
      !aligned16(y) || (bias != nullptr && !aligned16(bias))) {
    set_error("gemm_bf16x3_p4: shape / alignment outside the kernel's contract");
    return DRIN_E_UNSUPPORTED;
  }
  const int nx = (int)cdiv(N, x3p::BN);
  const int64_t tiles = cdiv(M, x3p::BM) * nx;
  if (tiles > ((int64_t)1 << 28)) return DRIN_E_UNSUPPORTED;
  unsigned full;
  int ksplit;
  tail_split_256(tiles, K / x3p::BK, tail, tail_floats, &full, &ksplit);
  const unsigned items = full + ((unsigned)tiles - full) * (unsigned)ksplit;
  static DynLdsOptIn opt;
  DRIN_TRY(ensure_dynamic_lds(opt, reinterpret_cast<const void*>(x3p::k_gemm_bf16x3_p4), x3p::p4::LDS, "hipFuncSetAttribute(gemm_bf16x3_p4)"));
  {
    KernelTimer timer(DRIN_KC_GEMM_X3, st);
    hipLaunchKernelGGL(x3p::k_gemm_bf16x3_p4, dim3(items), dim3(x3p::THREADS), x3p::p4::LDS, st, x, ldx, (const __bf16*)w_hi,
                       (const __bf16*)w_lo, ldw, bias, y, ldy, M, N, K, accumulate ? 1 : 0, nx, full, ksplit, tail);
    DRIN_CHECK_LAUNCH("k_gemm_bf16x3_p4");
  }
  if (ksplit > 1) DRIN_TRY(launch_tail_add_256(tail, y, ldy, M, N, (unsigned)nx, full, (unsigned)tiles - full, ksplit, st));
  return DRIN_OK;
}

int launch_gemm_x3_planes(const void* a_hi, const void* a_lo, int64_t lda, const void* b_hi, const void* b_lo,
                          int64_t ldb, const float* bias, float* y, int64_t ldy, int64_t M, int N, int K,
                          hipStream_t st, float* splitk, size_t splitk_floats) {
  if (M <= 0 || N <= 0) return DRIN_OK;
  const bool a_lo_plane = a_lo != nullptr;
  if (b_lo == nullptr) {
    set_error("gemm_x3_planes: the weight operand needs both planes");
    return DRIN_E_UNSUPPORTED;
  }
  if (K <= 0 || (K % x3p::BK) || (lda % 8) || (ldb % 8) || !aligned16(a_hi) || !aligned16(a_lo) || !aligned16(b_hi) ||
      !aligned16(b_lo)) {
    set_error("gemm_x3_planes: K=%d must be a multiple of 32, leading dimensions multiples of 8, planes 16-byte aligned", K);
    return DRIN_E_ALIGN;
  }
  const int64_t mt = cdiv(M, x3p::BM);
  if (mt > 65535) {
    set_error("gemm_x3_planes: %lld row tiles exceed the grid limit; split the batch", (long long)mt);
    return DRIN_E_SHAPE;
  }
  {
    static DynLdsOptIn opt_in[2];
    const void* kernels[2] = {reinterpret_cast<const void*>(x3p::k_gemm_x3_planes<true, true>),
                              reinterpret_cast<const void*>(x3p::k_gemm_x3_planes<false, true>)};
    for (int i = 0; i < 2; ++i)
      DRIN_TRY(ensure_dynamic_lds(opt_in[i], kernels[i], x3p::LDS_BYTES, "hipFuncSetAttribute(gemm_x3_planes)"));
  }
  int splits = 1;
  const int nkb = K / x3p::BK;
  const int64_t tiles = mt * cdiv(N, x3p::BN);
  if (splitk != nullptr && tiles <= 128 && (N % 4) == 0 && (ldy % 4) == 0 && aligned16(y) && aligned16(splitk)) {
    for (int s : {16, 8, 6, 4, 3, 2})
      if (tiles * s <= 256 && nkb % s == 0 && nkb / s >= 3 && (size_t)s * M * N <= splitk_floats) {
        splits = s;
        break;
      }
  }
  const int nx = (int)cdiv(N, x3p::BN);
  unsigned full = (unsigned)tiles;
  int ksplit = 1;
  if (splits == 1) tail_split_256(tiles, nkb, splitk, splitk_floats, &full, &ksplit);
  if ((a_lo_plane || tiles >= 128) && splits == 1 && (N % 4) == 0 && (ldy % 4) == 0 && aligned16(y) && (bias == nullptr || aligned16(bias))) {
    static DynLdsOptIn opt[2];
    auto kern = a_lo_plane ? x3p::k_gemm_x3_planes_p4<true, false> : x3p::k_gemm_x3_planes_p4<false, false>;
    DRIN_TRY(ensure_dynamic_lds(opt[a_lo_plane ? 0 : 1], reinterpret_cast<const void*>(kern), x3p::p4::LDS, "hipFuncSetAttribute(gemm_x3_planes_p4)"));
    const unsigned p4_items = full + ((unsigned)tiles - full) * (unsigned)ksplit;
    {
      KernelTimer timer(DRIN_KC_GEMM_PLANES, st);
      hipLaunchKernelGGL(kern, dim3(p4_items), dim3(x3p::THREADS), x3p::p4::LDS, st, (const __bf16*)a_hi,
                         (const __bf16*)(a_lo_plane ? a_lo : a_hi), lda, (const __bf16*)b_hi, (const __bf16*)b_lo, ldb, bias, y, ldy, M, N, K, nx,
                         full, ksplit, splitk, (const float*)nullptr, (const float*)nullptr);
      DRIN_CHECK_LAUNCH("k_gemm_x3_planes_p4");
    }
    if (ksplit > 1) DRIN_TRY(launch_tail_add_256(splitk, y, ldy, M, N, (unsigned)nx, full, (unsigned)tiles - full, ksplit, st));
    return DRIN_OK;
  }
  const unsigned items = full + ((unsigned)tiles - full) * (unsigned)ksplit;
  dim3 grid(items, 1, (unsigned)splits);
  const int64_t part_stride = M * (int64_t)N;
  float* out = splits > 1 ? splitk : y;
  {
    KernelTimer timer(DRIN_KC_GEMM_PLANES, st);
    const __bf16 *ah = (const __bf16*)a_hi, *al = (const __bf16*)a_lo, *bh = (const __bf16*)b_hi, *bl = (const __bf16*)b_lo;
    if (a_lo_plane)
      hipLaunchKernelGGL((x3p::k_gemm_x3_planes<true, true>), grid, dim3(x3p::THREADS), x3p::LDS_BYTES, st, ah, al, lda, bh,
                         bl, ldb, bias, out, ldy, M, N, K, part_stride, nx, full, ksplit, splitk);
    else
      hipLaunchKernelGGL((x3p::k_gemm_x3_planes<false, true>), grid, dim3(x3p::THREADS), x3p::LDS_BYTES, st, ah, al, lda, bh,
                         bl, ldb, bias, out, ldy, M, N, K, part_stride, nx, full, ksplit, splitk);
    DRIN_CHECK_LAUNCH("k_gemm_x3_planes");
  }
  if (splits > 1) DRIN_TRY(launch_splitk_reduce(splitk, splits, part_stride, bias, y, ldy, M, N, false, st));
  if (ksplit > 1) DRIN_TRY(launch_tail_add_256(splitk, y, ldy, M, N, (unsigned)nx, full, (unsigned)tiles - full, ksplit, st));
  return DRIN_OK;
}

bool gemm_f16_planes_fits(const void* a_f16, int64_t lda, const void* b_f16, int64_t ldb, const float* y, int64_t ldy, int64_t M, int N,
                          int K) {
  return cdiv(M, x3p::BM) * cdiv(N, x3p::BN) >= 128 && cdiv(M, x3p::BM) * cdiv(N, x3p::BN) <= ((int64_t)1 << 28) && K > 0 &&
         (K % (2 * x3p::BK)) == 0 && (lda % 8) == 0 && (ldb % 8) == 0 && (N % 4) == 0 && (ldy % 4) == 0 && aligned16(a_f16) &&
         aligned16(b_f16) && aligned16(y);
}

int launch_gemm_f16_planes(const void* a_f16, int64_t lda, const void* b_f16, int64_t ldb, const float* row_scale, const float* b_scale,
                           float* y, int64_t ldy, int64_t M, int N, int K, hipStream_t st, float* tail, size_t tail_floats) {
  if (M <= 0 || N <= 0) return DRIN_OK;
  if (row_scale == nullptr || b_scale == nullptr || !gemm_f16_planes_fits(a_f16, lda, b_f16, ldb, y, ldy, M, N, K)) {
    set_error("gemm_f16_planes: built for at least half a round of 256 x 256 tiles, K %% 64 == 0, 16-byte aligned planes and both scales");
    return DRIN_E_UNSUPPORTED;
  }
  const int nx = (int)cdiv(N, x3p::BN);
  const int64_t tiles = cdiv(M, x3p::BM) * nx;
  unsigned full;
  int ksplit;
  tail_split_256(tiles, K / (2 * x3p::BK), tail, tail_floats, &full, &ksplit);
  const unsigned items = full + ((unsigned)tiles - full) * (unsigned)ksplit;
  auto kern = x3p::k_gemm_x3_planes_p4<true, true>;
  static DynLdsOptIn opt;
  DRIN_TRY(ensure_dynamic_lds(opt, reinterpret_cast<const void*>(kern), x3p::p4::LDS, "hipFuncSetAttribute(gemm_f16_planes)"));
  {
    KernelTimer timer(DRIN_KC_GEMM_X3, st);
    hipLaunchKernelGGL(kern, dim3(items), dim3(x3p::THREADS), x3p::p4::LDS, st, (const __bf16*)a_f16, (const __bf16*)a_f16, lda,
                       (const __bf16*)b_f16, (const __bf16*)b_f16, ldb, (const float*)nullptr, y, ldy, M, N, K, nx, full, ksplit, tail, row_scale,
                       b_scale);
    DRIN_CHECK_LAUNCH("k_gemm_f16_planes");
  }
  if (ksplit > 1) DRIN_TRY(launch_tail_add_256(tail, y, ldy, M, N, (unsigned)nx, full, (unsigned)tiles - full, ksplit, st));
  return DRIN_OK;
}

}
```

drin_amd/csrc/internal.h:

```cpp
#pragma once
#include <hip/hip_runtime.h>
#include <stddef.h>
#include <stdint.h>

#include <atomic>

#include "../../include/drin_hip.h"

namespace drin {

void set_error(const char* fmt, ...);
int hip_fail(hipError_t e, const char* what);

#define DRIN_CHECK_LAUNCH(what)                                  \
  do {                                                           \
    hipError_t _e = hipGetLastError();                           \
    if (_e != hipSuccess) return ::drin::hip_fail(_e, what);     \
  } while (0)

#define DRIN_TRY(expr)              \
  do {                              \
    int _s = (expr);                \
    if (_s != DRIN_OK) return _s;   \
  } while (0)

struct KernelTimer {
  KernelTimer(int kernel_class, hipStream_t st);
  ~KernelTimer();
  int slot;
  hipStream_t stream;
};

struct DeviceScope {
  DeviceScope(void* stream, const void* device_pointer, const char* entry_point);
  ~DeviceScope();
  DeviceScope(const DeviceScope&) = delete;
  DeviceScope& operator=(const DeviceScope&) = delete;
  int status;
  int prev, dev, outer;
  bool switched;
};
int call_device();
#define DRIN_BIND_DEVICE(stream, device_pointer, entry_point)               \
  ::drin::DeviceScope _device_scope((stream), (device_pointer), (entry_point)); \
  if (_device_scope.status != DRIN_OK) return _device_scope.status

struct DynLdsOptIn {
  std::atomic<int> bytes[64] = {};
};
inline int ensure_dynamic_lds(DynLdsOptIn& s, const void* kernel, int bytes, const char* what) {
  const int dev = call_device();
  std::atomic<int>& mark = s.bytes[dev & 63];
  if (mark.load(std::memory_order_relaxed) >= bytes) return DRIN_OK;
  hipError_t e = hipFuncSetAttribute(kernel, hipFuncAttributeMaxDynamicSharedMemorySize, bytes);
  if (e != hipSuccess) return hip_fail(e, what);
  mark.store(bytes, std::memory_order_relaxed);
  return DRIN_OK;
}

struct RoctxRange {
  explicit RoctxRange(const char* name);
  ~RoctxRange();
  bool pushed;
};

inline bool aligned16(const void* p) { return (reinterpret_cast<uintptr_t>(p) & 15u) == 0; }
inline int64_t cdiv(int64_t a, int64_t b) { return (a + b - 1) / b; }
inline dim3 pair_grid(int B, int N) {
  return (B > 1 && B <= 65535) ? dim3((unsigned)cdiv(N, 4), (unsigned)B) : dim3((unsigned)cdiv((int64_t)B * N, 4));
}

int launch_axis_mean(const float* in, float* out, int64_t groups, int inner, int cols, hipStream_t st);
int launch_span_mean(const float* seq, const int64_t* start, const int64_t* end, float* out, int B, int L, int D,
                     hipStream_t st);
int launch_axis_mean_bf16(const void* in, float* out, int64_t groups, int inner, int cols, hipStream_t st);
int launch_span_mean_bf16(const void* seq, const int64_t* start, const int64_t* end, float* out, int B, int L, int D,
                          hipStream_t st);
int launch_entity_token_mean(const float* feat, const int64_t* mask, float* out, int64_t pairs, int T, int D,
                             hipStream_t st);
int launch_entity_token_mean_bf16(const void* feat, const int64_t* mask, float* out, int64_t pairs, int T, int D,
                                  hipStream_t st);
int launch_cosine_rows(const float* x, const float* y, int64_t y_stride, float* out, int B, int N, int D, float eps,
                       float scale, hipStream_t st, const int64_t* y_index = nullptr, const float* sim1 = nullptr,
                       const float* sim2 = nullptr, float* out1 = nullptr, float* out2 = nullptr, float div = 1.0f);
int launch_miei(const float* mobj, const float* mscore, const float* eobj, const float* escore, float* out, int B,
                int N, int Km, int Ke, int R, float cos_eps, float miei_eps, float scale, hipStream_t st,
                const int64_t* e_index = nullptr);
int launch_scale_div(const float* in, float* out, int64_t n, float mul, float div, hipStream_t st);

struct SliceSum {
  static constexpr int MAX_DST = 32, MAX_SEG = 40;
  struct Dst {
    float* y;
    int64_t ldy;
    int rows, c4;
    unsigned first_block;
    int seg_head, seg_tail;
  } dst[MAX_DST];
  struct Seg {
    const float* partial;
    int slices, next;
  } seg[MAX_SEG];
  int n = 0, n_seg = 0;
  int add(float* y, int64_t ldy, int rows, int cols, const float* partial, int slices);
};
int launch_slice_sum(SliceSum& s, hipStream_t st);

int launch_gemm_nt(const float* x, int64_t ldx, const float* w, int64_t ldw, const float* bias, float* y, int64_t ldy,
                   int64_t M, int N, int K, bool accumulate, int precision, hipStream_t st, float* splitk = nullptr,
                   size_t splitk_floats = 0, const float* w_planes = nullptr);
int launch_gemm_nt_bf16x3(const float* x, int64_t ldx, const float* w, int64_t ldw, const float* bias, float* y,
                          int64_t ldy, int64_t M, int N, int K, hipStream_t st, const void* w_hi = nullptr,
                          const void* w_lo = nullptr, bool accumulate = false,
                          float* tail = nullptr, size_t tail_floats = 0, const int64_t* a_index = nullptr);
int launch_to_f16_scaled(const float* x, void* out, int64_t n, float* scale, hipStream_t st);
bool gemm_tn_bf16x3_fits(int64_t lda, int64_t ldb, int64_t M, int N, int K, const void* a, const void* b);
int launch_gemm_tn_bf16x3(const float* a, int64_t lda, const float* b, int64_t ldb, float* y, int64_t ldy, int64_t M,
                          int N, int K, hipStream_t st, float* scratch, size_t scratch_floats,
                          const int64_t* b_index = nullptr);
bool gemm_tn_bf16x3_scratch_ok(const float* y, int64_t ldy, int N, int K, const float* scratch, size_t scratch_floats);
struct TnGroup {
  static constexpr int MAX = 8;
  struct Item {
    const float* a;
    int64_t lda;
    const float* b;
    int64_t ldb;
    float* y;
    int64_t ldy, M;
    int N, K;
    const int64_t* b_index;
    float* colsum;
  } item[MAX];
  int n = 0;
  int add(const float* a, int64_t lda, const float* b, int64_t ldb, float* y, int64_t ldy, int64_t M, int N, int K,
          const int64_t* b_index = nullptr, float* colsum = nullptr);
};
int launch_gemm_tn_group(const TnGroup& g, hipStream_t st, float* scratch, size_t scratch_floats, SliceSum* defer = nullptr);
int launch_gemm_x3_planes(const void* a_hi, const void* a_lo, int64_t lda, const void* b_hi, const void* b_lo,
                          int64_t ldb, const float* bias, float* y, int64_t ldy, int64_t M, int N, int K,
                          hipStream_t st, float* splitk = nullptr, size_t splitk_floats = 0);
bool gemm_f16_planes_fits(const void* a_f16, int64_t lda, const void* b_f16, int64_t ldb, const float* y, int64_t ldy, int64_t M, int N, int K);
int launch_gemm_f16_planes(const void* a_f16, int64_t lda, const void* b_f16, int64_t ldb, const float* row_scale, const float* b_scale,
                           float* y, int64_t ldy, int64_t M, int N, int K, hipStream_t st, float* tail = nullptr, size_t tail_floats = 0);
int launch_gemm_nt_bf16x3_p4(const float* x, int64_t ldx, const void* w_hi, const void* w_lo, int64_t ldw, const float* bias,
                             float* y, int64_t ldy, int64_t M, int N, int K, hipStream_t st, bool accumulate, float* tail = nullptr,
                             size_t tail_floats = 0);
int launch_tail_add_256(const float* tail, float* y, int64_t ldy, int64_t M, int N, unsigned col_tiles, unsigned full,
                        unsigned tail_tiles, int ksplit, hipStream_t st);
int launch_splitk_reduce(const float* partial, int splits, int64_t part_stride, const float* bias, float* y, int64_t ldy,
                         int64_t M, int N, bool accumulate, hipStream_t st);
int launch_split_planes(const float* x, void* hi, void* lo, int64_t n, hipStream_t st);
struct SplitBatch {
  const float* src[32];
  float* planes[32];
  int64_t n4[32];
  int n = 0;
  int add(const float* w, float* planes_out, int64_t numel);
};
int launch_split_planes_batch(const SplitBatch& b, hipStream_t st);
int launch_transpose_split_batch(const SplitBatch& b, int rows, int cols, hipStream_t st);
int launch_transpose(const float* in, float* out, int rows, int cols, hipStream_t st);
struct WtForms {
  const float* planes = nullptr;
  float* scratch = nullptr;
  size_t scratch_floats = 0;
  float* tail = nullptr;
  size_t tail_floats = 0;
};
bool gemm_nn_takes_bf16x3(int precision, int64_t M, int N, int K);
int launch_gemm_nn(const float* x, int64_t ldx, const float* w, int64_t ldw, float* y, int64_t ldy, int64_t M, int N,
                   int K, bool accumulate, int precision, hipStream_t st, float* splitk = nullptr, size_t splitk_floats = 0,
                   const WtForms& wt = WtForms());
struct F32GemmGroup {
  static constexpr int MAX = 8;
  struct Item {
    const float* a;
    int64_t lda;
    const float* b;
    int64_t ldb;
    float* y;
    int64_t ldy, M;
    int N, K;
  } item[MAX];
  const float* bias_of[MAX];
  int n = 0;
  int add_tn(const float* a, int64_t lda, const float* b, int64_t ldb, float* y, int64_t ldy, int64_t M, int N, int K);
  int add_nt(const float* x, int64_t ldx, const float* w, int64_t ldw, const float* bias, float* y, int64_t ldy, int64_t M, int N, int K);
};
int launch_gemm_tn_f32_group(const F32GemmGroup& g, hipStream_t st, float* scratch, size_t scratch_floats, SliceSum* defer = nullptr);
inline int small_tn_slices(int64_t reduction_rows) {
  const int64_t s = (reduction_rows + 127) / 128;
  return (int)(s > 4 ? 4 : (s < 1 ? 1 : s));
}
bool gemm_nt_f32_group_fits(const float* x, int64_t ldx, const float* w, int64_t ldw, const float* y, int64_t ldy, int64_t M, int N,
                            int K, int precision);
int launch_gemm_nt_f32_group(const F32GemmGroup& g, hipStream_t st, float* scratch, size_t scratch_floats);
struct NtProduct {
  const float *x, *w, *bias;
  float* y;
  int64_t ldx, ldw, ldy, rows;
  int n_out, k_red;
  const float* planes;
};
int launch_gemm_nt_pair(const NtProduct& a, const NtProduct& b, int precision, hipStream_t st, float* splitk, size_t splitk_floats);
int launch_gemm_tn(const float* a, int64_t lda, const float* b, int64_t ldb, float* y, int64_t ldy, int64_t M, int N,
                   int K, int precision, hipStream_t st, float* scratch = nullptr, size_t scratch_floats = 0);
enum TnKernel { TN_BF16X3, TN_F32_SMALL, TN_F32_LARGE };
TnKernel gemm_tn_kernel(int precision, const float* a, int64_t lda, const float* b, int64_t ldb, const float* y, int64_t ldy,
                        int64_t M, int N, int K, const float* scratch, size_t scratch_floats);

int launch_mention_aggregate(const float* e1, const float* v1, const float* e2, const float* v2, const float* u,
                             float* out, int B, int N, int D, hipStream_t st);
int launch_entity_aggregate(const float* e1, const float* m1, const float* e2, const float* m2, const float* v,
                            float* out, int B, int N, int D, hipStream_t st);
int launch_layer_aggregate(const float* e, int64_t edge_stride, const float* vm, const float* ve, float* agg_m,
                           float* agg_e, int B, int N, int D, bool live_image, hipStream_t st);
int launch_layernorm_gelu(const float* h, const float* gamma, const float* beta, float* y, float* mean, float* rstd,
                          int64_t rows, int D, float eps, hipStream_t st, int act = DRIN_ACT_GELU);
int launch_layernorm_gelu2(const float* h, float* y, float* mean, float* rstd, int64_t rows, const float* h2, float* y2,
                           float* mean2, float* rstd2, int64_t rows2, const float* gamma, const float* beta, int D, float eps,
                           hipStream_t st, int act = DRIN_ACT_GELU);
int launch_edge_update4(const float* fu, const float* fv, const float* e, float* out, int B, int N, int D,
                        hipStream_t st, int act = DRIN_ACT_SIGMOID, float* z_out = nullptr);

int launch_cosine_bwd(const float* x, const float* y, const float* g, float* dx, float* dy, float* scratch3, int B,
                      int N, int D, float eps, hipStream_t st);
int launch_layernorm_gelu_bwd(const float* h, const float* mean, const float* rstd, const float* gamma,
                              const float* beta, float* g, float* dgamma, float* dbeta, float* dbias, float* partial,
                              int64_t rows, int D, hipStream_t st, int act = DRIN_ACT_GELU);
int launch_layernorm_gelu_bwd2(const float* h, const float* mean, const float* rstd, float* g, int64_t rows, const float* h2,
                               const float* mean2, const float* rstd2, float* g2, int64_t rows2, const float* gamma,
                               const float* beta, float* dgamma, float* dbeta, float* dbias, float* partial, int D,
                               hipStream_t st, int act = DRIN_ACT_GELU, SliceSum* defer = nullptr, float* level1_own = nullptr);
constexpr int kColsumMaxSlices = 64;
int launch_colsum(const float* x, float* out, int64_t rows, int C, hipStream_t st, float* scratch = nullptr,
                  size_t scratch_floats = 0);
struct ColsumBatch {
  const float* x[8];
  float* out[8];
  int64_t rows[8];
  int c4[8];
  int by[8];
  int n = 0;
  int add(const float* src, float* dst, int64_t nrows, int C);
};
int launch_colsum_batch(const ColsumBatch& b, hipStream_t st, float* scratch, size_t scratch_floats, SliceSum* defer = nullptr);
int launch_edge_update_bwd(const float* g, const float* e_new, const float* fu, float* dpre, float* dfv, int B, int N, int D,
                           float scale, hipStream_t st, int act = DRIN_ACT_SIGMOID);
int launch_sigmoid_bwd(const float* g, const float* e_new, float* dpre, int64_t n, hipStream_t st, int act = DRIN_ACT_SIGMOID);
int launch_mention_reduce(const float* w1, const float* v1, const float* w2, const float* v2, const float* u,
                          float* out, int B, int N, int D, float scale, hipStream_t st);
int launch_mention_reduce2(const float* w, const float* v1, const float* v2, const float* uA, const float* uB,
                           float* outA, float* outB, int B, int N, int D, float scale, hipStream_t st);
int launch_mention_reduce2_pair(const float* wa, const float* va1, const float* va2, const float* uaA, const float* uaB, float* outaA,
                                float* outaB, float scale_a, const float* wb, const float* vb1, const float* vb2, const float* ubA,
                                const float* ubB, float* outbA, float* outbB, float scale_b, int B, int N, int D, hipStream_t st);
int launch_entity_combine(const float* w1, const float* m1, const float* w2, const float* m2, float* out, int B, int N,
                          int D, float scale, hipStream_t st);
int launch_entity_side_bwd(const float* dA_mt, const float* dA_mi, const float* dA_et, const float* dA_ei,
                           const float* mt, const float* mi, const float* et, const float* ei, const float* e,
                           const float* de_extra, float* d_et, float* d_ei, float* de, int B, int N, int D,
                           const float* mask, bool accumulate, hipStream_t st);

int launch_span_mean_bwd(const float* g, const int64_t* start, const int64_t* end, float* out, int B, int L, int D,
                         hipStream_t st);
int launch_axis_mean_bwd(const float* in, float* out, int64_t groups, int inner, int cols, hipStream_t st);
int launch_token_block_bwd(const float* g_pool, const float* g_cls, const int64_t* mask, void* out, int64_t pairs, int T,
                           int D, bool bf16, hipStream_t st);
int launch_row_sum(const float* in, float* out, int64_t rows, int C, hipStream_t st);
size_t miei_bwd_scratch_floats(int64_t pairs, int B, int Km, int Ke);
int launch_miei_bwd(const float* mobj, const float* mscore, const float* eobj, const float* escore, const float* g,
                    float* d_mobj, float* d_mscore, float* d_eobj, float* d_escore, float* scratch, int B, int N, int Km,
                    int Ke, int R, float cos_eps, float miei_eps, hipStream_t st);

int launch_expand_edges(const float* es, float* out, int64_t pairs4, int D, hipStream_t st);
int launch_mention_reduce_vec(const float* w1, const float* v1, const float* w2, const float* v2, const float* u,
                              float* out, int B, int N, int D, float scale, bool mean_style, hipStream_t st);
int launch_entity_aggregate_vec(const float* e1, const float* m1, const float* e2, const float* m2, const float* v,
                                float* out, int B, int N, int D, hipStream_t st);
int launch_edge_pre_vec(const float* fu, const float* fv, const float* e, float* pre, int B, int N, int D,
                        hipStream_t st);
int launch_sigmoid_inplace(float* x, int64_t n, hipStream_t st, int act = DRIN_ACT_SIGMOID, float* z_out = nullptr);
int launch_edge_pre_vec_bwd(const float* dpre, float* dfu, float* dfv, int B, int N, int D, hipStream_t st);
int launch_entity_side_bwd_vec(const float* dA_mt, const float* dA_mi, const float* dA_et, const float* dA_ei,
                               const float* mt, const float* mi, const float* et, const float* ei, const float* e,
                               const float* de_extra, float* d_et, float* d_ei, float* de, int B, int N, int D,
                               const float* mask, hipStream_t st);

struct WeightGradPass {
  struct Scratch { float* p; size_t floats; };
  const int prec;
  const bool vec;
  const hipStream_t st;
  const Scratch tn, small, colsum;
  int add(const float* dy, int64_t lddy, const float* x, int64_t ldx, float* dw, int64_t lddw, int64_t rows, int n_out,
          int k_red, const int64_t* x_index = nullptr, float* db = nullptr);
  SliceSum ln_sums;
  int flush_bias_sums() { const int rc = launch_colsum_batch(bias_sums, st, colsum.p, colsum.floats); bias_sums = ColsumBatch(); return rc; }
  void layers_done() { layer_sums = bias_sums.n, layer_small = dw_small.n, layer_group = dw_group.n; }
  int finish(void* layers_ready_event);
  ColsumBatch bias_sums;
  F32GemmGroup dw_small;
  TnGroup dw_group;
  int layer_sums = 0, layer_small = 0, layer_group = 0;
};
size_t small_group_worst_case_floats(const drin_config& c, size_t tn_part_floats);

}
```

include/drin_hip.h:

```cpp
#ifndef DRIN_HIP_H_
#define DRIN_HIP_H_

#include <stddef.h>
#include <stdint.h>

#ifdef __cplusplus
extern "C" {
#endif

#define DRIN_ABI_VERSION 12
#define DRIN_API __attribute__((visibility("default")))

typedef enum {
  DRIN_OK = 0,
  DRIN_E_SHAPE = -1,
  DRIN_E_NULL = -2,
  DRIN_E_ALIGN = -3,
  DRIN_E_WORKSPACE = -4,
  DRIN_E_HIP = -5,
  DRIN_E_UNSUPPORTED = -6,
  DRIN_E_INDEX = -7
} drin_status;

typedef enum {
  DRIN_PREC_F32 = 0,
  DRIN_PREC_BF16X3 = 1,
  DRIN_PREC_BF16X3_ALL = 3,
  DRIN_PREC_BF16X3_IF16 = 5
} drin_precision;

typedef struct {
  int32_t batch;
  int32_t num_candidates;
  int32_t embed_dim;
  int32_t image_dim;
  int32_t mention_tokens;
  int32_t image_regions;
  int32_t mention_objects;
  int32_t entity_objects;
  int32_t entity_tokens;
  int32_t mention_object_inner;
  int32_t entity_image_inner;
  int32_t entity_object_inner;
  int32_t num_layers;
  int32_t dynamic_edges;
  float edge_enabled[4];
  float layer_norm_eps;
  float cosine_eps;
  float miei_eps;
  float clip_scale;
  int32_t precision;
  int32_t num_entities;
  int32_t vector_edges;
  int32_t feature_dtype;
  int32_t vertex_activation;
  int32_t edge_activation;
  int32_t cache_format;
} drin_config;

typedef enum {
  DRIN_CACHE_F32 = 0,
  DRIN_CACHE_MIXED_F16 = 1
} drin_cache_format;

typedef enum {
  DRIN_ACT_DEFAULT = 0,
  DRIN_ACT_GELU = 1,
  DRIN_ACT_SIGMOID = 2,
  DRIN_ACT_RELU = 3,
  DRIN_ACT_TANH = 4,
  DRIN_ACT_SILU = 5
} drin_activation;

typedef enum {
  DRIN_FEAT_F32 = 0,
  DRIN_FEAT_BF16 = 1
} drin_feature_dtype;

typedef struct {
  const float* mention_text;
  const int64_t* mention_start;
  const int64_t* mention_end;
  const float* mention_image;
  const float* mention_object;
  const float* mention_object_score;
  const float* entity_text;
  const int64_t* entity_text_mask;
  const float* entity_image;
  const float* entity_object;
  const float* entity_object_score;
  const float* miet_similarity;
  const float* mtei_similarity;
  const int64_t* entity_index;
  const float* entity_text_cls;
  int32_t* index_status;
} drin_batch;

typedef struct {
  const float *w_h, *b_h, *w_u, *b_u, *w_v, *b_v, *ln_weight, *ln_bias;
  const float *w_m, *b_m;
} drin_layer_params;

#define DRIN_MAX_LAYERS 8

typedef struct {
  const float *w_mention_text, *b_mention_text;
  const float *w_entity_text, *b_entity_text;
  const float *w_mention_image, *b_mention_image;
  const float *w_entity_image, *b_entity_image;
  drin_layer_params layer[DRIN_MAX_LAYERS];
} drin_params;

typedef struct {
  float *w_mention_text, *b_mention_text, *w_entity_text, *b_entity_text;
  float *w_mention_image, *b_mention_image, *w_entity_image, *b_entity_image;
  struct { float *w_h, *b_h, *w_u, *b_u, *w_v, *b_v, *ln_weight, *ln_bias, *w_m, *b_m; } layer[DRIN_MAX_LAYERS];
} drin_param_grads;

typedef struct {
  float *mention_text, *mention_image, *mention_object, *mention_object_score;
  float *entity_text, *entity_text_cls, *entity_image, *entity_object, *entity_object_score;
  float *miet_similarity, *mtei_similarity;
  void* scratch;
  size_t scratch_bytes;
} drin_input_grads;

typedef struct {
  float* mention_text_vertex[DRIN_MAX_LAYERS + 1];
  float* mention_image_vertex[DRIN_MAX_LAYERS + 1];
  float* entity_text_vertex[DRIN_MAX_LAYERS + 1];
  float* entity_image_vertex[DRIN_MAX_LAYERS + 1];
  float* edges[DRIN_MAX_LAYERS + 1];
} drin_trace;

DRIN_API int drin_version(void);
DRIN_API const char* drin_last_error(void);
DRIN_API const char* drin_build_info(void);

DRIN_API int drin_default_config(drin_config* cfg);

DRIN_API int drin_host_selftest(void);

DRIN_API size_t drin_workspace_bytes(const drin_config* cfg, int for_training);


DRIN_API int drin_edges_fwd(const drin_config* cfg, const drin_batch* batch, float* edges, float* span_mean,
                   void* stream);

DRIN_API int drin_pool_fwd(const drin_config* cfg, const drin_batch* batch, float* pooled_entity_text,
                  float* pooled_mention_image, float* pooled_entity_image, void* stream);

DRIN_API int drin_linear_fwd(const float* x, const float* w, const float* bias, float* y, int64_t rows,
                    int32_t n_out, int32_t k, int32_t precision, void* stream);

DRIN_API int drin_linear_bwd(const float* x, const float* w, const float* dy, float* dx, float* dw, float* db,
                             int64_t rows, int32_t n_out, int32_t k, int32_t precision, float* scratch,
                             size_t scratch_floats, void* stream);

DRIN_API int drin_forward(const drin_config* cfg, const drin_batch* batch, const drin_params* params,
                 void* workspace, size_t workspace_bytes, float* scores, int keep_for_backward,
                 const drin_trace* trace, void* stream);

DRIN_API int drin_indexed_supported(const drin_config* cfg);

DRIN_API int drin_forward_staged(const drin_config* cfg, const drin_batch* batch, const drin_params* params,
                 void* workspace, size_t workspace_bytes, float* scores, int keep_for_backward,
                 const drin_trace* trace, void* params_ready_event, void* stream);

DRIN_API int drin_backward(const drin_config* cfg, const drin_batch* batch, const drin_params* params,
                  void* workspace, size_t workspace_bytes, const float* grad_scores,
                  const drin_param_grads* grads, void* stream);

DRIN_API int drin_backward_staged(const drin_config* cfg, const drin_batch* batch, const drin_params* params,
                  void* workspace, size_t workspace_bytes, const float* grad_scores,
                  const drin_param_grads* grads, void* layers_ready_event, void* stream);

DRIN_API int drin_backward_ex(const drin_config* cfg, const drin_batch* batch, const drin_params* params,
                              void* workspace, size_t workspace_bytes, const float* grad_scores,
                              const drin_param_grads* grads, const drin_input_grads* input_grads,
                              void* layers_ready_event, void* stream);
DRIN_API size_t drin_input_grad_scratch_bytes(const drin_config* cfg);

DRIN_API int drin_pool_bwd(const drin_config* cfg, const int64_t* entity_text_mask, const float* grad_pooled,
                           const float* grad_cls, void* grad_entity_text, void* stream);

DRIN_API int drin_fused_supported(const drin_config* cfg);
DRIN_API size_t drin_prepared_bytes(const drin_config* cfg);
DRIN_API size_t drin_fused_workspace_bytes(const drin_config* cfg);
DRIN_API int drin_prepare(const drin_config* cfg, const drin_params* params, void* prepared, size_t prepared_bytes,
                          void* stream);
DRIN_API int drin_forward_prepared(const drin_config* cfg, const drin_batch* batch, const drin_params* params,
                                   const void* prepared, void* workspace, size_t workspace_bytes, float* scores,
                                   void* stream);
DRIN_API int32_t drin_workgroups_per_mention(const drin_config* cfg, int32_t cached);

DRIN_API int32_t drin_image_contraction_passes(const drin_config* cfg, int32_t indexed);

DRIN_API int drin_index_status(int32_t* index_status, void* stream);

DRIN_API size_t drin_entity_cache_bytes(const drin_config* cfg);
DRIN_API size_t drin_entity_cache_build_workspace_bytes(const drin_config* cfg);
DRIN_API size_t drin_cached_workspace_bytes(const drin_config* cfg);
DRIN_API int drin_build_entity_cache(const drin_config* cfg, const drin_batch* tables, const drin_params* params,
                                     const void* prepared, void* cache, size_t cache_bytes, void* workspace,
                                     size_t workspace_bytes, void* stream);
DRIN_API int drin_forward_cached(const drin_config* cfg, const drin_batch* batch, const drin_params* params,
                                 const void* prepared, const void* cache, void* workspace, size_t workspace_bytes,
                                 float* scores, void* stream);

DRIN_API int drin_split_planes(const float* x, void* hi, void* lo, int64_t n, void* stream);
DRIN_API int drin_linear_planes_fwd(const void* x_hi, const void* x_lo, const void* w_hi, const void* w_lo,
                                    const float* bias, float* y, int64_t rows, int32_t n_out, int32_t k,
                                    void* stream);

DRIN_API size_t drin_loss_workspace_bytes(int32_t batch);
DRIN_API int drin_triplet_topk(const float* scores, const uint8_t* answer, int32_t batch, int32_t num_candidates,
                               float margin, const int32_t* topk, int32_t num_topk, float* loss, float* d_scores,
                               int64_t* correct, void* workspace, size_t workspace_bytes, void* stream);

DRIN_API int drin_adam_step(float* param, const float* grad, float* exp_avg, float* exp_avg_sq, int64_t n,
                            float lerp_weight, float beta2, float one_minus_beta2, float bias_correction2_sqrt, float eps,
                            float neg_step_size, void* stream);

typedef struct {
  int32_t batch;
  int32_t num_candidates;
  int32_t embed_dim;
  int32_t image_dim;
  int32_t mention_tokens;
  int32_t image_regions;
  int32_t precision;
  float cosine_eps;
  float thres_tmim;
  float thres_imie;
} drin_melhi_config;

typedef struct {
  const float* mention_feature;
  const int64_t* mention_mask;
  const int64_t* start;
  const int64_t* end;
  const float* mention_image;
  const float* entity_feature;
  const float* entity_image;
} drin_melhi_batch;

typedef struct {
  const float *w_image_map_text, *b_image_map_text;
  const float *w_ih, *w_hh, *b_ih, *b_hh;
  const float *w_mention_final_map, *b_mention_final_map;
  const float *w_entity_final_map, *b_entity_final_map;
} drin_melhi_params;

typedef struct {
  float *w_image_map_text, *b_image_map_text;
  float *w_ih, *w_hh, *b_ih, *b_hh;
  float *w_mention_final_map, *b_mention_final_map;
  float *w_entity_final_map, *b_entity_final_map;
} drin_melhi_param_grads;

DRIN_API size_t drin_melhi_workspace_bytes(const drin_melhi_config* cfg, int for_training);

DRIN_API int drin_melhi_forward(const drin_melhi_config* cfg, const drin_melhi_batch* batch, const drin_melhi_params* params,
                                const int32_t* order, const int32_t* lengths, void* workspace, size_t workspace_bytes,
                                float* scores, void* stream);
DRIN_API int drin_melhi_backward(const drin_melhi_config* cfg, const drin_melhi_batch* batch, const drin_melhi_params* params,
                                 const int32_t* order, const int32_t* lengths, void* workspace, size_t workspace_bytes,
                                 const float* grad_scores, const drin_melhi_param_grads* grads, void* stream);

typedef struct {
  int32_t batch;
  int32_t num_candidates;
  int32_t embed_dim;
  int32_t image_dim;
  int32_t mention_tokens;
  int32_t image_regions;
  int32_t num_heads;
  int32_t entity_tokens;
  int32_t precision;
  float layer_norm_eps;
  float cosine_eps;
} drin_ghmfc_config;

typedef struct {
  const float* mention_feature;
  const int64_t* mention_mask;
  const float* mention_image;
  const float* entity_feature;
  const int64_t* entity_mask;
} drin_ghmfc_batch;

typedef struct {
  const float *a2b_wq, *a2b_wk, *a2b_wv;
  const float *a2b_in_bias;
  const float *a2b_wo, *a2b_bo;
  const float *a2b_ffn_w, *a2b_ffn_b;
  const float *b2a_in_w, *b2a_in_bias;
  const float *b2a_wo, *b2a_bo;
  const float *b2a_ffn_w, *b2a_ffn_b;
  const float *ln0_w, *ln0_b, *ln1_w, *ln1_b, *ln2_w, *ln2_b, *ln3_w, *ln3_b;
} drin_ghmfc_cross_params;

typedef struct {
  drin_ghmfc_cross_params t2v;
  drin_ghmfc_cross_params v2t;
  const float *w_text_linear, *b_text_linear;
  const float *w_image_linear, *b_image_linear;
  const float *w_score_linear, *b_score_linear;
  const float *w_entity, *b_entity;
} drin_ghmfc_params;

DRIN_API size_t drin_ghmfc_workspace_bytes(const drin_ghmfc_config* cfg);

DRIN_API int drin_ghmfc_forward(const drin_ghmfc_config* cfg, const drin_ghmfc_batch* batch, const drin_ghmfc_params* params,
                                void* workspace, size_t workspace_bytes, float* scores, float* mention_repr, void* stream);

DRIN_API int drin_attention(const float* q, int64_t ldq, const float* k, int64_t ldk, const float* v, int64_t ldv,
                            const int64_t* key_mask, float* out, int64_t ldo, int32_t batch, int32_t num_heads, int32_t q_len,
                            int32_t k_len, int32_t head_dim, void* stream);

DRIN_API int drin_attention_train_fwd(const float* q, int64_t ldq, const float* k, int64_t ldk, const float* v, int64_t ldv,
                                      const int64_t* key_mask, float* out, int64_t ldo, float* lse, int32_t batch,
                                      int32_t num_heads, int32_t q_len, int32_t k_len, int32_t head_dim, void* stream);

DRIN_API int drin_attention_bwd(const float* q, int64_t ldq, const float* k, int64_t ldk, const float* v, int64_t ldv,
                                const int64_t* key_mask, const float* out, int64_t ldo, const float* lse, const float* dout,
                                int64_t lddo, float* dq, int64_t lddq, float* dk, int64_t lddk, float* dv, int64_t lddv,
                                float* delta_scratch, int32_t batch, int32_t num_heads, int32_t q_len, int32_t k_len,
                                int32_t head_dim, void* stream);


typedef enum {
  DRIN_KC_GEMM = 0,
  DRIN_KC_POOL = 1,
  DRIN_KC_EDGE = 2,
  DRIN_KC_GCN = 3,
  DRIN_KC_STREAM = 4,
  DRIN_KC_GEMM_X3 = 5,
  DRIN_KC_GEMM_PLANES = 6,
  DRIN_KC_OPTIM = 7,
  DRIN_KC_LSTM = 8,
  DRIN_KC_CELL = 9,
  DRIN_KC_ATTN = 10,
  DRIN_KC_NORM = 11,
  DRIN_KC_COUNT = 12
} drin_kernel_class;

DRIN_API int drin_profile_begin(int max_launches);
DRIN_API int drin_profile_end(double* ms_by_class, int64_t* launches_by_class);
DRIN_API const char* drin_kernel_class_name(int kernel_class);

#ifdef __cplusplus
}
#endif
#endif
```

Before: 26.02 million pairs/s.

## Overlap image-candidate GEMM rows on a side stream with the mention head

Moves about 90% of the row tiles of the large entity-image contraction onto a per-device side stream. There it runs as a persistent kernel with few workgroups, concurrently with the serial mention-side head and layer GEMMs. The main stream waits on a join event, then finishes the remaining row tiles and the split-K tail. This is meant to fill idle compute units during the small, latency-bound mention stages, at the cost of contention between streams, extra event syncs, and a path that is skipped under graph capture.

```diff
diff --git a/drin_amd/_lib.py b/drin_amd/_lib.py
--- a/drin_amd/_lib.py
+++ b/drin_amd/_lib.py
@@ -150,6 +150,7 @@
     "drin_workgroups_per_mention": (C.c_int32, [C.POINTER(DrinConfigC), C.c_int32]),
     "drin_index_status": (C.c_int, [C.c_void_p, C.c_void_p]),
     "drin_image_contraction_passes": (C.c_int32, [C.POINTER(DrinConfigC), C.c_int32]),
+    "drin_image_contraction_side_tiles": (C.c_int32, [C.POINTER(DrinConfigC), C.c_int32]),
     "drin_prepare": (C.c_int, [C.POINTER(DrinConfigC), C.POINTER(DrinParamsC), C.c_void_p, C.c_size_t, C.c_void_p]),
     "drin_forward_prepared": (C.c_int, [C.POINTER(DrinConfigC), C.POINTER(DrinBatchC), C.POINTER(DrinParamsC), C.c_void_p,
                                         C.c_void_p, C.c_size_t, C.c_void_p, C.c_void_p]),
diff --git a/drin_amd/csrc/api.hip b/drin_amd/csrc/api.hip
--- a/drin_amd/csrc/api.hip
+++ b/drin_amd/csrc/api.hip
@@ -77,6 +77,30 @@
   if (status != DRIN_OK || prev < 0) return;
   g_call_device = outer;
   if (switched) (void)hipSetDevice(prev);
+}
+
+static SideLane g_side_lanes[64];
+static std::mutex g_side_lanes_mutex;
+
+int side_lane(SideLane** out) {
+  const int dev = call_device();
+  if (dev < 0 || dev >= 64) {
+    set_error("side stream: device %d outside the 64 the library keeps state for", dev);
+    return DRIN_E_UNSUPPORTED;
+  }
+  SideLane& lane = g_side_lanes[dev];
+  if (!lane.ready.load(std::memory_order_acquire)) {
+    std::lock_guard<std::mutex> lock(g_side_lanes_mutex);
+    if (!lane.ready.load(std::memory_order_relaxed)) {
+      hipError_t e = hipStreamCreateWithFlags(&lane.stream, hipStreamNonBlocking);
+      if (e == hipSuccess) e = hipEventCreateWithFlags(&lane.fork, hipEventDisableTiming);
+      if (e == hipSuccess) e = hipEventCreateWithFlags(&lane.join, hipEventDisableTiming);
+      if (e != hipSuccess) return hip_fail(e, "side stream of the device");
+      lane.ready.store(true, std::memory_order_release);
+    }
+  }
+  *out = &lane;
+  return DRIN_OK;
 }
 
 struct Roctx {
diff --git a/drin_amd/csrc/fused_forward.hip b/drin_amd/csrc/fused_forward.hip
--- a/drin_amd/csrc/fused_forward.hip
+++ b/drin_amd/csrc/fused_forward.hip
@@ -74,6 +74,63 @@
          cdiv(M, 256) * cdiv(c->embed_dim, 256) >= 128;
 }
 
+#ifndef DRIN_SIDE_WGS
+#define DRIN_SIDE_WGS 64
+#endif
+#ifndef DRIN_SIDE_PERMILLE
+#define DRIN_SIDE_PERMILLE 900
+#endif
+#ifndef DRIN_SIDE_MIN_TILES
+#define DRIN_SIDE_MIN_TILES 1200
+#endif
+constexpr int kSideWgs = DRIN_SIDE_WGS;
+constexpr int kSidePermille = DRIN_SIDE_PERMILLE;
+constexpr int64_t kSideMinTiles = DRIN_SIDE_MIN_TILES;
+#ifdef DRIN_SIDE_PROBE
+static int g_probe_wgs = kSideWgs, g_probe_permille = kSidePermille;
+extern "C" __attribute__((visibility("default"))) void drin_probe_side_plan(int wgs, int permille) { g_probe_wgs = wgs, g_probe_permille = permille; }
+#endif
+struct SidePlan {
+  int64_t S = 0;
+  int G = 0;
+};
+static SidePlan image_side_plan(const drin_config* c, bool indexed, bool capturing) {
+  SidePlan plan;
+  int wgs = kSideWgs, permille = kSidePermille;
+#ifdef DRIN_SIDE_PROBE
+  wgs = g_probe_wgs, permille = g_probe_permille;
+#endif
+  const bool split = c->precision == DRIN_PREC_BF16X3 || c->precision == DRIN_PREC_BF16X3_ALL || c->precision == DRIN_PREC_BF16X3_IF16;
+  if (capturing || indexed || !split || if16_gate(c, indexed) || wgs <= 0 || permille <= 0) return plan;
+  const int D = c->embed_dim, R = c->image_dim;
+  if ((D % 32) || (R % 32) || c->batch <= 0) return plan;
+  const int64_t M = (int64_t)c->batch * c->num_candidates;
+  const int64_t nx = cdiv(D, 256), row_tiles = cdiv(M, 256), tiles = row_tiles * nx;
+  if (tiles < 192 || tiles < kSideMinTiles || tiles > ((int64_t)1 << 28)) return plan;
+  FusedLayout L;
+  L.build(*c);
+  const int64_t whole_rows = gemm_p4_whole_tiles(tiles, R, L.splitk_floats > 0, L.splitk_floats) / nx;
+  int64_t S = (row_tiles * permille + 500) / 1000;
+  S = S < whole_rows ? S : whole_rows;
+  S = S < row_tiles - 1 ? S : row_tiles - 1;
+  if (S <= 0) return plan;
+  plan.S = S;
+  plan.G = (int)(wgs < S * nx ? wgs : S * nx);
+  return plan;
+}
+
+struct SideJoin {
+  SideLane* lane = nullptr;
+  hipStream_t st = nullptr;
+  int join() {
+    if (!lane) return DRIN_OK;
+    const hipError_t e = hipStreamWaitEvent(st, lane->join, 0);
+    lane = nullptr;
+    return e == hipSuccess ? DRIN_OK : hip_fail(e, "hipStreamWaitEvent(side stream)");
+  }
+  ~SideJoin() { (void)join(); }
+};
+
 int fused_supported(const drin_config* c) {
   if (c->num_layers != 2) {
     set_error("fused path: built for num_layers == 2 (got %d); use drin_forward", c->num_layers);
@@ -283,6 +340,13 @@
   const bool indexed = b->entity_index != nullptr;
   const bool xi_planes = planes && indexed;
   const bool if16 = if16_gate(cfg, indexed) && gemm_f16_planes_fits(ws + L.p_xi, R, pb + P.p_cimg_f16, R, ws + L.h_image, D, M, D, R);
+  hipStreamCaptureStatus capture = hipStreamCaptureStatusNone;
+  if (hipStreamIsCapturing(st, &capture) != hipSuccess) {
+    (void)hipGetLastError();
+    capture = hipStreamCaptureStatusActive;
+  }
+  SidePlan side = image_side_plan(cfg, indexed, capture != hipStreamCaptureStatusNone);
+  if (!aligned16(b->entity_image) || !aligned16(ws + L.h_image) || !b->entity_image) side = SidePlan();
   if (b->entity_text_cls) {
     set_error("drin_forward_prepared: entity_text_cls (text pooled ahead of time) is a form of the training entry points");
     return DRIN_E_UNSUPPORTED;
@@ -312,6 +376,29 @@
   float* vm0 = ws + L.vm0;
   float* hmfu = ws + L.hmfu;
   const bool xt_exact = bf16_feat && !tokens;
+  const GemmScratch psk = L.pair_splitk_floats ? GemmScratch{ws + L.pair_splitk, L.pair_splitk_floats} : msk;
+  auto image_rows_product = [&](hipStream_t on, RowTiles rows) -> int {
+    const __bf16* ci = reinterpret_cast<const __bf16*>(pb + P.p_cimg);
+    if (bf16_feat)
+      return launch_gemm_x3_planes(b->entity_image, nullptr, R, ci, ci + (size_t)D * R, R, nullptr, ws + L.h_image, D, M, D, R, on, psk.p,
+                                   psk.floats, rows);
+    return launch_gemm_nt_bf16x3_p4((const float*)b->entity_image, R, ci, ci + (size_t)D * R, R, nullptr, ws + L.h_image, D, M, D, R, on, false,
+                                    aligned16(psk.p) ? psk.p : nullptr, psk.floats, rows);
+  };
+  SideJoin side_join;
+  if (side.S > 0) {
+    SideLane* lane = nullptr;
+    DRIN_TRY(side_lane(&lane));
+    std::lock_guard<std::mutex> order(lane->order);
+    hipError_t e = hipEventRecord(lane->fork, st);
+    if (e == hipSuccess) e = hipStreamWaitEvent(lane->stream, lane->fork, 0);
+    if (e != hipSuccess) return hip_fail(e, "fork to the side stream");
+    const int rc = image_rows_product(lane->stream, RowTiles{0, side.S, side.G});
+    e = hipEventRecord(lane->join, lane->stream);
+    side_join.lane = lane, side_join.st = st;
+    if (rc != DRIN_OK) return rc;
+    if (e != hipSuccess) return hip_fail(e, "hipEventRecord(side stream)");
+  }
   DRIN_TRY(run_folded_head(cfg, b, params, pb, P, planes, ws + L.span_mean, ws + L.mimg, vm0, hmfu, msk, st));
   if (dyn)
     DRIN_TRY(launch_gemm_nt(hmfu + D, 2 * D, pb + P.ecat, D, nullptr, ws + L.q, D + R, 2 * (int64_t)B, D + R, D, false, prec, st, msk.p,
@@ -369,7 +456,6 @@
   float* vm1 = ws + L.vm1;
   DRIN_TRY(launch_gemm_nt(ws + L.agg1, D, L1.w_h, D, L1.b_h, vm1, D, 2 * (int64_t)B, D, D, false, prec, st, msk.p, msk.floats, wp(P.p_wh1)));
   DRIN_TRY(run_folded_mention_finish(cfg, params, pb, P, planes, vm1, ws + L.hm2, msk, st));
-  const GemmScratch psk = L.pair_splitk_floats ? GemmScratch{ws + L.pair_splitk, L.pair_splitk_floats} : msk;
   if (planes) {
     const __bf16* ct = reinterpret_cast<const __bf16*>(pb + P.p_ctxt);
     const __bf16* ci = reinterpret_cast<const __bf16*>(pb + P.p_cimg);
@@ -381,7 +467,10 @@
     else if (xi_planes)
       DRIN_TRY(launch_gemm_x3_planes(xi_hi, bf16_feat ? nullptr : xi_hi + MR, R, ci, ci + (size_t)D * R, R, nullptr, ws + L.h_image, D, M,
                                      D, R, st, psk.p, psk.floats));
-    else if (bf16_feat)
+    else if (side.S > 0) {
+      DRIN_TRY(side_join.join());
+      DRIN_TRY(image_rows_product(st, RowTiles{side.S, -1, 0}));
+    } else if (bf16_feat)
       DRIN_TRY(launch_gemm_x3_planes(b->entity_image, nullptr, R, ci, ci + (size_t)D * R, R, nullptr, ws + L.h_image, D, M, D, R, st, psk.p,
                                      psk.floats));
     else
@@ -428,6 +517,11 @@
   return L.chunks;
 }
 
+int32_t drin_image_contraction_side_tiles(const drin_config* cfg, int32_t indexed) {
+  if (validate_config(cfg) != DRIN_OK || fused_supported(cfg) != DRIN_OK) return 0;
+  return (int32_t)image_side_plan(cfg, indexed != 0, false).S;
+}
+
 int32_t drin_image_contraction_passes(const drin_config* cfg, int32_t indexed) {
   if (validate_config(cfg) != DRIN_OK || fused_supported(cfg) != DRIN_OK) return 0;
   if (cfg->precision == DRIN_PREC_F32) return 0;
diff --git a/drin_amd/csrc/gemm_x3_planes.hip b/drin_amd/csrc/gemm_x3_planes.hip
--- a/drin_amd/csrc/gemm_x3_planes.hip
+++ b/drin_amd/csrc/gemm_x3_planes.hip
@@ -2,6 +2,7 @@
 
 #include "device_utils.h"
 #include "internal.h"
+#include "tile_walk.h"
 
 namespace drin {
 
@@ -16,19 +17,16 @@
 constexpr int BUF_BYTES = 4 * PLANE_BYTES;
 constexpr int LDS_BYTES = 2 * BUF_BYTES;
 
-__device__ __forceinline__ void tile_of_block(int& tile_x, int64_t& tile_y, int nx, unsigned full, int ksplit, int& kpart,
-                                              unsigned& tail_slot) {
-  const unsigned id = blockIdx.x;
+__device__ __forceinline__ void tile_of_block(unsigned id, unsigned tile0, int& tile_x, int64_t& tile_y, int nx, unsigned full, int ksplit,
+                                              int& kpart, unsigned& tail_slot) {
   unsigned t;
   kpart = 0;
   tail_slot = 0;
   if (id < full) {
-    const unsigned xcd = id & 7, k = id >> 3;
-    const unsigned q = full >> 3, rem = full & 7;
-    t = (xcd < rem ? xcd * (q + 1) : rem * (q + 1) + (xcd - rem) * q) + k;
+    t = tile0 + xcd_tile_of_item(id, full);
   } else {
     const unsigned u = id - full;
-    t = full + u / (unsigned)ksplit;
+    t = tile0 + full + u / (unsigned)ksplit;
     kpart = (int)(u % (unsigned)ksplit);
     tail_slot = (u / (unsigned)ksplit) * (unsigned)(ksplit - 1) + (unsigned)(kpart - 1);
   }
@@ -107,7 +105,7 @@
   int tx, kpart;
   int64_t ty;
   unsigned tail_slot;
-  tile_of_block(tx, ty, nx, full, ksplit, kpart, tail_slot);
+  tile_of_block(blockIdx.x, 0u, tx, ty, nx, full, ksplit, kpart, tail_slot);
   const int64_t m0 = ty * BM;
   const int n0 = tx * BN;
   if (blockIdx.x >= full) {
@@ -232,13 +230,13 @@
 
 }
 
-template <bool A_LO = true, bool F16 = false>
-__global__ void __launch_bounds__(THREADS, 2)
-    k_gemm_x3_planes_p4(const __bf16* __restrict__ a_hi, const __bf16* __restrict__ a_lo, int64_t lda,
-                        const __bf16* __restrict__ b_hi, const __bf16* __restrict__ b_lo, int64_t ldb,
-                        const float* __restrict__ bias, float* __restrict__ C, int64_t ldc, int64_t M, int N, int K, int nx,
-                        unsigned full, int ksplit, float* __restrict__ tail, const float* __restrict__ row_scale,
-                        const float* __restrict__ b_scale) {
+template <bool A_LO, bool F16>
+__device__ __forceinline__ void p4_planes_item(char* smem, unsigned id, unsigned tile0, const __bf16* __restrict__ a_hi,
+                                               const __bf16* __restrict__ a_lo, int64_t lda, const __bf16* __restrict__ b_hi,
+                                               const __bf16* __restrict__ b_lo, int64_t ldb, const float* __restrict__ bias,
+                                               float* __restrict__ C, int64_t ldc, int64_t M, int N, int K, int nx, unsigned full, int ksplit,
+                                               float* __restrict__ tail, const float* __restrict__ row_scale,
+                                               const float* __restrict__ b_scale) {
   static_assert(!F16 || A_LO, "the fp16 form uses both slots of every unit");
   constexpr int KSTEP = F16 ? 2 * BK : BK;
   constexpr int KB_BYTES = KSTEP * 2;
@@ -246,15 +244,14 @@
     a_lo = a_hi + BK;
     b_lo = b_hi + BK;
   }
-  extern __shared__ __attribute__((aligned(16))) char smem[];
   int tx, kpart;
   int64_t ty;
   unsigned tail_slot;
-  tile_of_block(tx, ty, nx, full, ksplit, kpart, tail_slot);
+  tile_of_block(id, tile0, tx, ty, nx, full, ksplit, kpart, tail_slot);
   const int64_t m0 = ty * BM;
   const int n0 = tx * BN;
   int64_t k0 = 0;
-  if (blockIdx.x >= full) {
+  if (id >= full) {
     K /= ksplit;
     k0 = (int64_t)kpart * K;
   }
@@ -427,6 +424,23 @@
     }
 }
 
+template <bool A_LO = true, bool F16 = false, bool PERSIST = false>
+__global__ void __launch_bounds__(THREADS, 2)
+    k_gemm_x3_planes_p4(const __bf16* __restrict__ a_hi, const __bf16* __restrict__ a_lo, int64_t lda,
+                        const __bf16* __restrict__ b_hi, const __bf16* __restrict__ b_lo, int64_t ldb,
+                        const float* __restrict__ bias, float* __restrict__ C, int64_t ldc, int64_t M, int N, int K, int nx,
+                        unsigned full, int ksplit, float* __restrict__ tail, const float* __restrict__ row_scale,
+                        const float* __restrict__ b_scale, unsigned tile0) {
+  extern __shared__ __attribute__((aligned(16))) char smem[];
+  if (PERSIST) {
+    for (unsigned id = blockIdx.x; id < full; id += gridDim.x)
+      p4_planes_item<A_LO, F16>(smem, id, tile0, a_hi, a_lo, lda, b_hi, b_lo, ldb, bias, C, ldc, M, N, K, nx, full, 1, tail, row_scale, b_scale);
+  } else {
+    p4_planes_item<A_LO, F16>(smem, blockIdx.x, tile0, a_hi, a_lo, lda, b_hi, b_lo, ldb, bias, C, ldc, M, N, K, nx, full, ksplit, tail, row_scale,
+                              b_scale);
+  }
+}
+
 
 typedef float f32x4v __attribute__((ext_vector_type(4)));
 typedef __bf16 bf16x4p __attribute__((ext_vector_type(4)));
@@ -438,18 +452,17 @@
   *reinterpret_cast<bf16x4p*>(hi_plane + 128 * 64 + off) = l;
 }
 
-__global__ void __launch_bounds__(THREADS, 2)
-    k_gemm_bf16x3_p4(const float* __restrict__ A, int64_t lda, const __bf16* __restrict__ b_hi, const __bf16* __restrict__ b_lo,
-                     int64_t ldb, const float* __restrict__ bias, float* __restrict__ C, int64_t ldc, int64_t M, int N, int K,
-                     int accumulate, int nx, unsigned full, int ksplit, float* __restrict__ tail) {
-  extern __shared__ __attribute__((aligned(16))) char smem[];
+__device__ __forceinline__ void p4_f32a_item(char* smem, unsigned id, unsigned tile0, const float* __restrict__ A, int64_t lda,
+                                            const __bf16* __restrict__ b_hi, const __bf16* __restrict__ b_lo, int64_t ldb,
+                                            const float* __restrict__ bias, float* __restrict__ C, int64_t ldc, int64_t M, int N, int K,
+                                            int accumulate, int nx, unsigned full, int ksplit, float* __restrict__ tail) {
   int tx, kpart;
   int64_t ty;
   unsigned tail_slot;
-  tile_of_block(tx, ty, nx, full, ksplit, kpart, tail_slot);
+  tile_of_block(id, tile0, tx, ty, nx, full, ksplit, kpart, tail_slot);
   const int64_t m0 = ty * BM;
   const int n0 = tx * BN;
-  if (blockIdx.x >= full) {
+  if (id >= full) {
     K /= ksplit;
     const int64_t k0 = (int64_t)kpart * K;
     A += k0;
@@ -670,6 +683,20 @@
     }
 }
 
+template <bool PERSIST = false>
+__global__ void __launch_bounds__(THREADS, 2)
+    k_gemm_bf16x3_p4(const float* __restrict__ A, int64_t lda, const __bf16* __restrict__ b_hi, const __bf16* __restrict__ b_lo,
+                     int64_t ldb, const float* __restrict__ bias, float* __restrict__ C, int64_t ldc, int64_t M, int N, int K,
+                     int accumulate, int nx, unsigned full, int ksplit, float* __restrict__ tail, unsigned tile0) {
+  extern __shared__ __attribute__((aligned(16))) char smem[];
+  if (PERSIST) {
+    for (unsigned id = blockIdx.x; id < full; id += gridDim.x)
+      p4_f32a_item(smem, id, tile0, A, lda, b_hi, b_lo, ldb, bias, C, ldc, M, N, K, accumulate, nx, full, 1, tail);
+  } else {
+    p4_f32a_item(smem, blockIdx.x, tile0, A, lda, b_hi, b_lo, ldb, bias, C, ldc, M, N, K, accumulate, nx, full, ksplit, tail);
+  }
+}
+
 __global__ void __launch_bounds__(256) k_split_planes(const float* __restrict__ x, __bf16* __restrict__ hi,
                                                       __bf16* __restrict__ lo, int64_t n4) {
   const int64_t i = (int64_t)blockIdx.x * 256 + threadIdx.x;
@@ -779,9 +806,38 @@
     }
 }
 
+int64_t gemm_p4_whole_tiles(int64_t tiles, int K, bool tail_scratch, size_t tail_floats) {
+  alignas(16) static const float some_scratch[4] = {0.f, 0.f, 0.f, 0.f};
+  unsigned full;
+  int ksplit;
+  tail_split_256(tiles, K / x3p::BK, tail_scratch ? some_scratch : nullptr, tail_floats, &full, &ksplit);
+  return (int64_t)full;
+}
+
+struct SliceItems {
+  unsigned tile0, whole;
+  bool with_tail;
+};
+static int slice_items(const RowTiles& rows, int64_t row_tiles, int nx, unsigned full, SliceItems* out) {
+  const int64_t begin = rows.begin, end = rows.end < 0 ? row_tiles : rows.end;
+  if (begin < 0 || end > row_tiles || begin > end || rows.wgs < 0) {
+    set_error("gemm p4: row tiles [%lld, %lld) outside the product's %lld", (long long)begin, (long long)end, (long long)row_tiles);
+    return DRIN_E_SHAPE;
+  }
+  out->with_tail = end == row_tiles && rows.wgs == 0;
+  const int64_t last = end == row_tiles ? (int64_t)full : end * nx;
+  if (begin * nx > (int64_t)full || last > (int64_t)full || (end == row_tiles && rows.wgs > 0 && (int64_t)full != row_tiles * nx)) {
+    set_error("gemm p4: a slice of row tiles must lie in the product's whole tiles (the tail split goes with the last plain launch)");
+    return DRIN_E_UNSUPPORTED;
+  }
+  out->tile0 = (unsigned)(begin * nx);
+  out->whole = (unsigned)(last - begin * nx);
+  return DRIN_OK;
+}
+
 int launch_gemm_nt_bf16x3_p4(const float* x, int64_t ldx, const void* w_hi, const void* w_lo, int64_t ldw, const float* bias,
                              float* y, int64_t ldy, int64_t M, int N, int K, hipStream_t st, bool accumulate, float* tail,
-                             size_t tail_floats) {
+                             size_t tail_floats, RowTiles rows) {
   if (M <= 0 || N <= 0) return DRIN_OK;
   if (K <= 0 || (K % x3p::BK) || (ldx % 4) || (ldw % 8) || (N % 4) || (ldy % 4) || !aligned16(x) || !aligned16(w_hi) || !aligned16(w_lo) ||
       !aligned16(y) || (bias != nullptr && !aligned16(bias))) {
@@ -794,23 +850,28 @@
   unsigned full;
   int ksplit;
   tail_split_256(tiles, K / x3p::BK, tail, tail_floats, &full, &ksplit);
-  const unsigned items = full + ((unsigned)tiles - full) * (unsigned)ksplit;
-  static DynLdsOptIn opt;
-  DRIN_TRY(ensure_dynamic_lds(opt, reinterpret_cast<const void*>(x3p::k_gemm_bf16x3_p4), x3p::p4::LDS, "hipFuncSetAttribute(gemm_bf16x3_p4)"));
+  SliceItems sl;
+  DRIN_TRY(slice_items(rows, cdiv(M, x3p::BM), nx, full, &sl));
+  static DynLdsOptIn opt[2];
+  auto kern = rows.wgs > 0 ? x3p::k_gemm_bf16x3_p4<true> : x3p::k_gemm_bf16x3_p4<false>;
+  DRIN_TRY(ensure_dynamic_lds(opt[rows.wgs > 0 ? 1 : 0], reinterpret_cast<const void*>(kern), x3p::p4::LDS, "hipFuncSetAttribute(gemm_bf16x3_p4)"));
+  const unsigned items = rows.wgs > 0 ? (unsigned)rows.wgs : sl.whole + (sl.with_tail ? ((unsigned)tiles - full) * (unsigned)ksplit : 0u);
+  if (items == 0 || sl.whole + (sl.with_tail ? (unsigned)tiles - full : 0u) == 0) return DRIN_OK;
   {
     KernelTimer timer(DRIN_KC_GEMM_X3, st);
-    hipLaunchKernelGGL(x3p::k_gemm_bf16x3_p4, dim3(items), dim3(x3p::THREADS), x3p::p4::LDS, st, x, ldx, (const __bf16*)w_hi,
-                       (const __bf16*)w_lo, ldw, bias, y, ldy, M, N, K, accumulate ? 1 : 0, nx, full, ksplit, tail);
+    hipLaunchKernelGGL(kern, dim3(items), dim3(x3p::THREADS), x3p::p4::LDS, st, x, ldx, (const __bf16*)w_hi, (const __bf16*)w_lo, ldw, bias, y,
+                       ldy, M, N, K, accumulate ? 1 : 0, nx, sl.whole, ksplit, tail, sl.tile0);
     DRIN_CHECK_LAUNCH("k_gemm_bf16x3_p4");
   }
-  if (ksplit > 1) DRIN_TRY(launch_tail_add_256(tail, y, ldy, M, N, (unsigned)nx, full, (unsigned)tiles - full, ksplit, st));
+  if (ksplit > 1 && sl.with_tail) DRIN_TRY(launch_tail_add_256(tail, y, ldy, M, N, (unsigned)nx, full, (unsigned)tiles - full, ksplit, st));
   return DRIN_OK;
 }
 
 int launch_gemm_x3_planes(const void* a_hi, const void* a_lo, int64_t lda, const void* b_hi, const void* b_lo,
                           int64_t ldb, const float* bias, float* y, int64_t ldy, int64_t M, int N, int K,
-                          hipStream_t st, float* splitk, size_t splitk_floats) {
+                          hipStream_t st, float* splitk, size_t splitk_floats, RowTiles rows) {
   if (M <= 0 || N <= 0) return DRIN_OK;
+  const bool sliced = rows.begin != 0 || rows.end >= 0 || rows.wgs != 0;
   const bool a_lo_plane = a_lo != nullptr;
   if (b_lo == nullptr) {
     set_error("gemm_x3_planes: the weight operand needs both planes");
@@ -848,19 +909,32 @@
   int ksplit = 1;
   if (splits == 1) tail_split_256(tiles, nkb, splitk, splitk_floats, &full, &ksplit);
   if ((a_lo_plane || tiles >= 128) && splits == 1 && (N % 4) == 0 && (ldy % 4) == 0 && aligned16(y) && (bias == nullptr || aligned16(bias))) {
-    static DynLdsOptIn opt[2];
-    auto kern = a_lo_plane ? x3p::k_gemm_x3_planes_p4<true, false> : x3p::k_gemm_x3_planes_p4<false, false>;
-    DRIN_TRY(ensure_dynamic_lds(opt[a_lo_plane ? 0 : 1], reinterpret_cast<const void*>(kern), x3p::p4::LDS, "hipFuncSetAttribute(gemm_x3_planes_p4)"));
-    const unsigned p4_items = full + ((unsigned)tiles - full) * (unsigned)ksplit;
+    SliceItems sl;
+    DRIN_TRY(slice_items(rows, mt, nx, full, &sl));
+    const bool persist = rows.wgs > 0;
+    if (persist && a_lo_plane) {
+      set_error("gemm_x3_planes: the persistent grid is built for an activation operand that is exact in bf16 (no lo plane)");
+      return DRIN_E_UNSUPPORTED;
+    }
+    static DynLdsOptIn opt[3];
+    auto kern = persist ? x3p::k_gemm_x3_planes_p4<false, false, true>
+                        : a_lo_plane ? x3p::k_gemm_x3_planes_p4<true, false, false> : x3p::k_gemm_x3_planes_p4<false, false, false>;
+    DRIN_TRY(ensure_dynamic_lds(opt[persist ? 2 : a_lo_plane ? 0 : 1], reinterpret_cast<const void*>(kern), x3p::p4::LDS, "hipFuncSetAttribute(gemm_x3_planes_p4)"));
+    const unsigned p4_items = persist ? (unsigned)rows.wgs : sl.whole + (sl.with_tail ? ((unsigned)tiles - full) * (unsigned)ksplit : 0u);
+    if (p4_items == 0 || sl.whole + (sl.with_tail ? (unsigned)tiles - full : 0u) == 0) return DRIN_OK;
     {
       KernelTimer timer(DRIN_KC_GEMM_PLANES, st);
       hipLaunchKernelGGL(kern, dim3(p4_items), dim3(x3p::THREADS), x3p::p4::LDS, st, (const __bf16*)a_hi,
                          (const __bf16*)(a_lo_plane ? a_lo : a_hi), lda, (const __bf16*)b_hi, (const __bf16*)b_lo, ldb, bias, y, ldy, M, N, K, nx,
-                         full, ksplit, splitk, (const float*)nullptr, (const float*)nullptr);
+                         sl.whole, ksplit, splitk, (const float*)nullptr, (const float*)nullptr, sl.tile0);
       DRIN_CHECK_LAUNCH("k_gemm_x3_planes_p4");
     }
-    if (ksplit > 1) DRIN_TRY(launch_tail_add_256(splitk, y, ldy, M, N, (unsigned)nx, full, (unsigned)tiles - full, ksplit, st));
+    if (ksplit > 1 && sl.with_tail) DRIN_TRY(launch_tail_add_256(splitk, y, ldy, M, N, (unsigned)nx, full, (unsigned)tiles - full, ksplit, st));
     return DRIN_OK;
+  }
+  if (sliced) {
+    set_error("gemm_x3_planes: a slice of row tiles runs on the four-phase kernel only (outside its contract here)");
+    return DRIN_E_UNSUPPORTED;
   }
   const unsigned items = full + ((unsigned)tiles - full) * (unsigned)ksplit;
   dim3 grid(items, 1, (unsigned)splits);
@@ -909,7 +983,7 @@
     KernelTimer timer(DRIN_KC_GEMM_X3, st);
     hipLaunchKernelGGL(kern, dim3(items), dim3(x3p::THREADS), x3p::p4::LDS, st, (const __bf16*)a_f16, (const __bf16*)a_f16, lda,
                        (const __bf16*)b_f16, (const __bf16*)b_f16, ldb, (const float*)nullptr, y, ldy, M, N, K, nx, full, ksplit, tail, row_scale,
-                       b_scale);
+                       b_scale, 0u);
     DRIN_CHECK_LAUNCH("k_gemm_f16_planes");
   }
   if (ksplit > 1) DRIN_TRY(launch_tail_add_256(tail, y, ldy, M, N, (unsigned)nx, full, (unsigned)tiles - full, ksplit, st));
diff --git a/drin_amd/csrc/internal.h b/drin_amd/csrc/internal.h
--- a/drin_amd/csrc/internal.h
+++ b/drin_amd/csrc/internal.h
@@ -4,6 +4,7 @@
 #include <stdint.h>
 
 #include <atomic>
+#include <mutex>
 
 #include "../../include/drin_hip.h"
 
@@ -44,6 +45,14 @@
 #define DRIN_BIND_DEVICE(stream, device_pointer, entry_point)               \
   ::drin::DeviceScope _device_scope((stream), (device_pointer), (entry_point)); \
   if (_device_scope.status != DRIN_OK) return _device_scope.status
+
+struct SideLane {
+  hipStream_t stream = nullptr;
+  hipEvent_t fork = nullptr, join = nullptr;
+  std::mutex order;
+  std::atomic<bool> ready{false};
+};
+int side_lane(SideLane** out);
 
 struct DynLdsOptIn {
   std::atomic<int> bytes[64] = {};
@@ -137,15 +146,20 @@
           const int64_t* b_index = nullptr, float* colsum = nullptr);
 };
 int launch_gemm_tn_group(const TnGroup& g, hipStream_t st, float* scratch, size_t scratch_floats, SliceSum* defer = nullptr);
+struct RowTiles {
+  int64_t begin = 0, end = -1;
+  int wgs = 0;
+};
+int64_t gemm_p4_whole_tiles(int64_t tiles, int K, bool tail_scratch, size_t tail_floats);
 int launch_gemm_x3_planes(const void* a_hi, const void* a_lo, int64_t lda, const void* b_hi, const void* b_lo,
                           int64_t ldb, const float* bias, float* y, int64_t ldy, int64_t M, int N, int K,
-                          hipStream_t st, float* splitk = nullptr, size_t splitk_floats = 0);
+                          hipStream_t st, float* splitk = nullptr, size_t splitk_floats = 0, RowTiles rows = RowTiles());
 bool gemm_f16_planes_fits(const void* a_f16, int64_t lda, const void* b_f16, int64_t ldb, const float* y, int64_t ldy, int64_t M, int N, int K);
 int launch_gemm_f16_planes(const void* a_f16, int64_t lda, const void* b_f16, int64_t ldb, const float* row_scale, const float* b_scale,
                            float* y, int64_t ldy, int64_t M, int N, int K, hipStream_t st, float* tail = nullptr, size_t tail_floats = 0);
 int launch_gemm_nt_bf16x3_p4(const float* x, int64_t ldx, const void* w_hi, const void* w_lo, int64_t ldw, const float* bias,
                              float* y, int64_t ldy, int64_t M, int N, int K, hipStream_t st, bool accumulate, float* tail = nullptr,
-                             size_t tail_floats = 0);
+                             size_t tail_floats = 0, RowTiles rows = RowTiles());
 int launch_tail_add_256(const float* tail, float* y, int64_t ldy, int64_t M, int N, unsigned col_tiles, unsigned full,
                         unsigned tail_tiles, int ksplit, hipStream_t st);
 int launch_splitk_reduce(const float* partial, int splits, int64_t part_stride, const float* bias, float* y, int64_t ldy,
diff --git a/drin_amd/csrc/tile_walk.h b/drin_amd/csrc/tile_walk.h
--- /dev/null
+++ b/drin_amd/csrc/tile_walk.h
@@ -0,0 +1,24 @@
+#pragma once
+
+#if defined(__HIPCC__) || defined(__CUDACC__)
+#define DRIN_TILE_WALK_FN __host__ __device__ __forceinline__
+#else
+#define DRIN_TILE_WALK_FN inline
+#endif
+
+namespace drin {
+namespace x3p {
+
+DRIN_TILE_WALK_FN unsigned xcd_tile_of_item(unsigned id, unsigned count) {
+  const unsigned xcd = id & 7, k = id >> 3;
+  const unsigned q = count >> 3, rem = count & 7;
+  return (xcd < rem ? xcd * (q + 1) : rem * (q + 1) + (xcd - rem) * q) + k;
+}
+
+DRIN_TILE_WALK_FN unsigned persistent_items(unsigned g, unsigned wgs, unsigned count) { return g < count ? (count - g + wgs - 1) / wgs : 0u; }
+DRIN_TILE_WALK_FN unsigned persistent_tile(unsigned g, unsigned wgs, unsigned i, unsigned count, unsigned tile0) {
+  return tile0 + xcd_tile_of_item(g + i * wgs, count);
+}
+
+}
+}
diff --git a/include/drin_hip.h b/include/drin_hip.h
--- a/include/drin_hip.h
+++ b/include/drin_hip.h
@@ -196,6 +196,8 @@
 
 DRIN_API int32_t drin_image_contraction_passes(const drin_config* cfg, int32_t indexed);
 
+DRIN_API int32_t drin_image_contraction_side_tiles(const drin_config* cfg, int32_t indexed);
+
 DRIN_API int drin_index_status(int32_t* index_status, void* stream);
 
 DRIN_API size_t drin_entity_cache_bytes(const drin_config* cfg);
```

New measurement: 27.93 million pairs/s (median of 6 runs). 1.07x the previous value.
